# nianticlabs/map-free-reloc

Measured on AMD Instinct MI355X. Metric: image-pairs/sec @ 540x720 (SuperPoint+SuperGlue + PnP w/ depth), higher is better.
Workload: dtype f32 in / f32 accumulate; matrix products of the 3x3 convolutions, attention, the transformer's linear layers and SuperPoint's 1x1 descriptor head on the f16 matrix cores with every fp32 operand carried as TWO f16 terms (xh = rne_f16(x), xl = rne_f16((x - xh) 2^11); weights pre-scaled per output feat

## Files before the change

include/mfr_hip.h:

```cpp
#ifndef MFR_HIP_H
#define MFR_HIP_H
#include <stddef.h>
#include <stdint.h>

#ifdef __cplusplus
extern "C" {
#endif

#define MFR_ABI_VERSION 6

#define MFR_K_F32 0
#define MFR_K_F64 1

#define MFR_E_ARG      (-1)
#define MFR_E_LAUNCH   (-2)
#define MFR_E_WORKSPACE (-3)

#define MFR_ST_OK          0
#define MFR_ST_TOO_FEW     1
#define MFR_ST_BAD_DEPTH   2
#define MFR_ST_NO_MODEL    3
#define MFR_ST_DEGENERATE  4

int mfr_abi_version(void);

int mfr_f16x2_guard_bind(int *device_flag);
#define MFR_ST_RANGE 7
const char *mfr_target_arch(void);

int mfr_test_f64_ops(const double *a, const double *b, const double *c, int n, double *out3, void *stream);
int mfr_test_sample(uint64_t seed, const int64_t *pair_ids, int B, int iters, int n, int k, int32_t *out, void *stream);

size_t mfr_pnp_workspace_bytes(int B, int maxN, int max_iters);
int mfr_pnp_solve_batch(const float *pts0, const float *pts1, const int32_t *n_corr, int B, int maxN,
                        const float *depth0, int H, int W,
                        const void *K0, const void *K1, int k_dtype,
                        int max_iters, double reproj_thr, double confidence,
                        uint64_t seed, const int64_t *pair_ids,
                        void *workspace, size_t workspace_bytes,
                        double *R, double *t, int32_t *n_inliers, int32_t *status, uint8_t *inlier_mask,
                        void *stream);

int mfr_depth_min(const float *depth, int B, int H, int W, float *partial_min , void *stream);
int mfr_pnp_lift(const float *pts0, const float *pts1, const int32_t *n_corr, int B, int maxN,
                 const float *depth0, const float *partial_min, int H, int W, const void *K0, int k_dtype,
                 double *xyz, double *obs, int32_t *src_idx, int32_t *n_valid, void *stream);
int mfr_pnp_ransac(const double *xyz, const double *obs, const int32_t *n_valid, int B, int maxN,
                   const void *K1, int k_dtype, int max_iters, double reproj_thr, double confidence,
                   uint64_t seed, const int64_t *pair_ids,
                   int32_t *counts , int32_t *inl_idx ,
                   double *R, double *t, int32_t *n_inliers, int32_t *status,
                   uint8_t *mask_valid ,
                   int32_t *best_iter , int32_t *iters_run ,
                   void *stream);

size_t mfr_rig_pnp_workspace_bytes(int B, int T, int maxN, int max_iters);
int mfr_rig_pnp_ransac(const double *xyz, const double *obs, const int32_t *n_valid, int B, int T, int maxN,
                       const void *K1, int k_dtype, const double *rig, int max_iters, double reproj_thr, double confidence,
                       uint64_t seed, const int64_t *pair_ids,
                       int32_t *counts , int32_t *inl_idx ,
                       double *R, double *t, int32_t *n_inliers, int32_t *status,
                       uint8_t *mask_valid ,
                       int32_t *best_iter , int32_t *iters_run ,
                       void *stream);
int mfr_rig_pnp_solve_batch(const float *pts0, const float *pts1, const int32_t *n_corr, int B, int T, int maxN,
                            const float *depth0, int H, int W,
                            const void *K0, const void *K1, int k_dtype, const double *rig,
                            int max_iters, double reproj_thr, double confidence,
                            uint64_t seed, const int64_t *pair_ids,
                            void *workspace, size_t workspace_bytes,
                            double *R, double *t, int32_t *n_inliers, int32_t *status, uint8_t *inlier_mask ,
                            void *stream);

size_t mfr_scale_workspace_bytes(int B, int maxN);
int mfr_scale_from_depth_batch(const float *pts0, const float *pts1, const uint8_t *emat_mask,
                               const int32_t *n_corr, int B, int maxN,
                               const float *depth0, const float *depth1, int H, int W,
                               const void *K0, const void *K1, int k_dtype,
                               const double *R, const double *t,
                               const int32_t *in_status ,
                               double scale_thr,
                               void *workspace, size_t workspace_bytes,
                               double *t_metric, double *best_scale, int32_t *n_inliers, int32_t *status,
                               void *stream);

#define MFR_AP_OK            0
#define MFR_AP_APPROXIMATED  1
#define MFR_AP_NO_PAIRS      2
#define MFR_AP_TOO_MANY      3
#define MFR_AP_BAD_OFFSETS   4
#define MFR_AP_ITER_CAP      16
#define MFR_AP_MAX_PAIRS     64
#define MFR_AP_MAX_LO_ITERS  62
#define MFR_AP_WEISZFELD_CAP 256
size_t mfr_abs_pose_workspace_bytes(int P);
int mfr_abs_pose_fuse(const double *train_q, const double *train_c, const double *pred_R, const double *pred_t, int P,
                      const int32_t *offsets, int Q, int mode, double thr_deg, double thr_mult, int lo_iters, uint64_t seed,
                      void *workspace, size_t workspace_bytes,
                      double *abs_q, double *abs_c, int32_t *inlier_mask, int32_t *status, void *stream);
int mfr_test_abs_pose_subset(uint64_t seed, const uint64_t *base, int n, int calls, int iters, int nsub, uint64_t *out, void *stream);

#define MFR_EMAT_SCORE_MAGSAC 0
#define MFR_EMAT_SCORE_COUNT  1
#define MFR_MAGSAC_LUT_M 2048
int mfr_magsac_lut(double *lut_host , int M);
size_t mfr_emat_workspace_bytes(int B, int maxN, int max_iters);
int mfr_emat_solve_batch(const float *pts0, const float *pts1, const int32_t *n_corr, int B, int maxN,
                         const void *K0, const void *K1, int k_dtype, double pix_thr, double confidence, int max_iters,
                         uint64_t seed, const int64_t *pair_ids, int score_method, const double *magsac_lut, int lut_m,
                         double max_thr_ratio, void *workspace, size_t workspace_bytes,
                         double *R, double *t, int32_t *n_inliers, int32_t *status, uint8_t *inlier_mask,
                         int32_t *best_iter, int32_t *iters_run, int32_t *counts_out, double *losses_out, int32_t *lo_runs,
                         void *stream);

size_t mfr_procrustes_workspace_bytes(int B, int maxN, int max_iters);
int mfr_procrustes_solve_batch(const float *pts0, const float *pts1, const int32_t *n_corr, int B, int maxN,
                               const float *depth0, const float *depth1, int H, int W, const void *K0, const void *K1, int k_dtype,
                               double max_corr_dist, double confidence, int max_iters, uint64_t seed, const int64_t *pair_ids,
                               void *workspace, size_t workspace_bytes, double *R, double *t, int32_t *n_inliers,
                               int32_t *status, int32_t *best_iter, int32_t *iters_run, int32_t *counts_out, void *stream);

int mfr_sp_scoremap(const float *logits, int B, int Hc, int Wc, float *scores, void *stream);
int mfr_sp_nms_candidates(const float *scores, int B, int H, int W, int nms_radius, float threshold, int border,
                          float *nms_out, uint64_t *cand, int cand_cap, int32_t *cand_count, void *stream);
int mfr_sp_select_topk(const uint64_t *cand, int cand_cap, const int32_t *cand_count, int B, int W, int K,
                       float *kpts, float *kscores, int32_t *n_kpts, void *stream);
int mfr_sp_sample_descriptors(const float *dense_nhwc, int B, int Hc, int Wc, const float *kpts,
                              const int32_t *n_kpts, int K, float *desc, void *stream);

size_t mfr_gemm_f16x2_pack_bytes(int N, int K);
int mfr_gemm_f16x2_pack(const float *w, int N, int K, void *packed, void *stream);
int mfr_gemm_f16x2(const float *x, int ldx, const void *packed_w, const float *bias, float *y, int ldy, int M, int N, int K, int flags, void *stream);
int mfr_gemm_f16x2_pack_batched(const float *w, int ldw, int nbatch, long long w_batch_stride, int N, int K, float out_mul, void *packed, void *stream);
int mfr_gemm_f16x2_batched(const float *x, int ldx, long long x_batch_stride, const void *packed_w, const float *bias, float *y, int ldy, long long y_batch_stride,
                           int nbatch, int M, int N, int K, int flags, void *stream);
int mfr_conv_igemm_k(int Cin, int KH, int KW);
int mfr_conv_igemm_f16x2(const float *x, const void *packed_w, const float *bias, float *y, int B, int Cin, int H, int W, int Cout, int KH, int KW,
                         int stride, int pad, int relu, void *stream);
int mfr_conv_igemm_f16x2_pad(const float *x, const void *packed_w, const float *bias, float *y, int B, int Cin, int H, int W, int Cout, int KH, int KW,
                             int stride, int pad_lo, int pad_hi, int relu, void *stream);
int mfr_conv_igemm_f16x2_upadd(const float *x, const void *packed_w, const float *bias, const float *lo, int Hl, int Wl, float *y, int B, int Cin, int H, int W,
                               int Cout, int KH, int KW, int stride, int pad, void *stream);
int mfr_gemm_f16x2_ln(const float *x, int ldx, const void *packed_w, const float *bias, const float *gamma, const float *beta, float eps, float *y, int ldy,
                      int M, int N, int K, int accumulate, void *stream);
int mfr_gemm_bf16x3_ln(const float *x, int ldx, const void *packed_w, const float *bias, const float *gamma, const float *beta, float eps, float *y, int ldy,
                       int M, int N, int K, int accumulate, void *stream);
int mfr_gemm_f16x2_windows(const float *feat, int Bimg, int Hf, int Wf, int C, const int32_t *img_ids, const int32_t *cell_ids, int nwin, int wc, int stride, int win,
                           const float *zero_row, const void *packed_w, const float *bias, const float *window_bias, float *y, int ldy, int N, void *stream);
int mfr_gemm_bf16x3_windows(const float *feat, int Bimg, int Hf, int Wf, int C, const int32_t *img_ids, const int32_t *cell_ids, int nwin, int wc, int stride, int win,
                            const float *zero_row, const void *packed_w, const float *bias, const float *window_bias, float *y, int ldy, int N, void *stream);
int mfr_mlp_ln_f16x2(const float *x, int ldx, int K1, const void *packed_w1, const float *b1, const void *packed_w2, const float *b2, const float *gamma, const float *beta,
                     float eps, float *y, int ldy, int M, int accumulate, void *stream);
int mfr_mlp_ln_bf16x3(const float *x, int ldx, int K1, const void *packed_w1, const float *b1, const void *packed_w2, const float *b2, const float *gamma, const float *beta,
                      float eps, float *y, int ldy, int M, int accumulate, void *stream);
size_t mfr_gemm_bf16x3_pack_bytes(int N, int K);
int mfr_gemm_bf16x3_pack(const float *w, int N, int K, void *packed, void *stream);
int mfr_gemm_bf16x3(const float *x, int ldx, const void *packed_w, const float *bias, float *y, int ldy, int M, int N, int K, int flags, void *stream);
int mfr_sg_attention(const float *q, const float *k, const float *v, int ld, int B2, int N, int heads,
                     const int32_t *n_tok, int cross, float *out, int ldo, void *stream);
int mfr_sg_attention_variant(const float *q, const float *k, const float *v, int ld, int B2, int N, int heads,
                             const int32_t *n_tok, int cross, float *out, int ldo, int variant, void *stream);
size_t mfr_sg_match_workspace_bytes(int B, int ldS);
int mfr_sg_sinkhorn_match(const float *S, int B, int ldS, const int32_t *n0, const int32_t *n1,
                          float bin_score, int iters, float match_thr,
                          const float *kpts0, const float *kpts1, int K,
                          void *workspace, size_t workspace_bytes,
                          int32_t *matches0, float *mscores0, float *pts0, float *pts1, int maxN, int32_t *n_corr,
                          void *stream);
int mfr_sg_sinkhorn_match_variant(const float *S, int B, int ldS, const int32_t *n0, const int32_t *n1,
                                  float bin_score, int iters, float match_thr,
                                  const float *kpts0, const float *kpts1, int K,
                                  void *workspace, size_t workspace_bytes,
                                  int32_t *matches0, float *mscores0, float *pts0, float *pts1, int maxN, int32_t *n_corr,
                                  int variant, void *stream);

int mfr_gemm_f16x2_ln_gelu(const float *x, int ldx, const void *packed_w, const float *bias, const float *gamma, const float *beta, float eps, float *y, int ldy,
                           int M, int N, int K, void *stream);
int mfr_gemm_bf16x3_ln_gelu(const float *x, int ldx, const void *packed_w, const float *bias, const float *gamma, const float *beta, float eps, float *y, int ldy,
                            int M, int N, int K, void *stream);
int mfr_lg_rotary_table(const float *kpts_norm, const float *wr, int M, float *cs, void *stream);
int mfr_lg_rotary_apply(float *q, float *k, int ld, int M, const float *cs, void *stream);
int mfr_lg_ln_gelu(float *x, int ld, int M, const float *gamma, const float *beta, float eps, void *stream);
size_t mfr_lg_assign_workspace_bytes(int B, int N0, int N1);
int mfr_lg_assign(const float *S, int B, int N0, int N1, int ldS, const float *z0, const float *z1, const int32_t *n0, const int32_t *n1,
                  float threshold, const float *kpts0, const float *kpts1, int K, void *workspace, size_t workspace_bytes,
                  int32_t *matches0, int32_t *matches1, float *mscores0, float *mscores1, float *pts0, float *pts1, int maxN, int32_t *n_corr,
                  void *stream);

size_t mfr_loftr_linear_attention_workspace_bytes(int B, int L, int heads);
int mfr_loftr_linear_attention(const float *q, int ldq, const float *k, const float *v, int ld, int B, int L, int heads,
                               void *workspace, size_t workspace_bytes, float *out, int ldo, void *stream);
int mfr_loftr_fine_attention(const float *q, int ldq, const float *k, const float *v, int ld, int Bw, int L, int D, int heads,
                             float *out, int ldo, void *stream);
size_t mfr_loftr_coarse_match_workspace_bytes(int B, int L0, int L1);
int mfr_loftr_coarse_match(const float *S, int B, int h0, int w0, int h1, int w1, float temperature, float thr, int border,
                           void *workspace, size_t workspace_bytes, int32_t *i_ids, int32_t *j_ids, float *mconf,
                           int32_t *n_match, void *stream);
int mfr_loftr_coarse_match_variant(const float *S, int B, int h0, int w0, int h1, int w1, float temperature, float thr, int border,
                                   void *workspace, size_t workspace_bytes, int32_t *i_ids, int32_t *j_ids, float *mconf,
                                   int32_t *n_match, int variant, void *stream);
size_t mfr_loftr_ot_match_workspace_bytes(int B, int L0, int L1);
int mfr_loftr_ot_match(const float *S, int B, int h0, int w0, int h1, int w1, float bin_score, int iters, float thr, int border,
                       void *workspace, size_t workspace_bytes, int32_t *i_ids, int32_t *j_ids, float *mconf, int32_t *n_match,
                       float *u_out, float *v_out, int variant, void *stream);
int mfr_loftr_gather_windows(const float *feat, int Bimg, int Hf, int Wf, int C, const int32_t *img_ids,
                             const int32_t *cell_ids, int M, int wc, int stride, int win, float *out, void *stream);
int mfr_loftr_fine_match(const float *g0, const float *g1, int ld, int C, int M, int W, float out_scale, const int32_t *lin_idx,
                         const float *k1, float *pts1, float *expec, void *stream);

int mfr_conv3x3_c1_relu(const float *x, const float *w, const float *bias, int B, int H, int W, int out_channels,
                        float *y, void *stream);
int mfr_bias_relu_nchw(float *x, const float *bias, int B, int C, int HW, void *stream);
int mfr_conv1x1_nchw(const float *x, const float *w, const float *bias, int B, int Cin, int Cout, int HW, float *y, void *stream);
int mfr_nchw_to_rows(const float *x, const float *add, int B, int C, int HW, int deinterleave, float *out, long long out_img_stride, int ldo, void *stream);
int mfr_nchw_to_rows_gather(const float *x, const float *add, int n_src, int C, int HW, const int32_t *idx, int n_out, float *out, long long out_img_stride,
                            int ldo, void *stream);
int mfr_bias_pool2_relu_nchw(const float *x, const float *bias, int B, int C, int H, int W, float *y, void *stream);

size_t mfr_procrustes_icp_workspace_bytes(int B, int H, int W);
int mfr_procrustes_icp_refine(const float *depth0, const float *depth1, int B, int H, int W, const void *K0, const void *K1, int k_dtype,
                              double max_corr_dist, double rel_fitness, double rel_rmse, int max_iter, const int32_t *status,
                              void *workspace, size_t workspace_bytes, double *R, double *t, int32_t *n_inliers, double *fitness,
                              double *rmse, int32_t *iters, void *stream);

int mfr_layernorm(const float *x, int ldx, const float *gamma, const float *beta, const float *residual, int ldr, long long rows, int C,
                  float eps, float *out, int ldo, void *stream);
int mfr_upsample2x_add(const float *lo, float *y, int planes, int H, int W, void *stream);
int mfr_upsample_bilinear(const void *in, void *out, int planes, int H, int W, int Ho, int Wo, int dtype, void *stream);
int mfr_conv_gemm_bf16(const void *A, long long sA, const long long *segA, const void *B, long long sB, const long long *segB,
                       int Lk, int nkc_total, int nkc_z, const float *bias, void *C, long long ldc, int out_dtype,
                       int M, int N, int nz, const long long *zA, const long long *zB, const long long *zC, const int *zk, void *stream);
int mfr_conv_pack_nhwc_halo(const void *x, int x_dtype, int B, int C, int H, int W, int Wp, void *out, int guard_rows, void *stream);
int mfr_conv_pack_cm_halo(const void *x, int x_dtype, long long BC, int H, int W, int Wq, long long L, int ncopies, int first_shift, long long slack,
                          void *out, void *stream);
int mfr_conv_unpack_nchw(const void *haloed, int B, int N, int H, int W, int Wp, void *y, void *stream);

int mfr_kabsch_fwd(const float *H, int B, float *R, void *stream);
int mfr_kabsch_bwd(const float *H, const float *gR, int B, float *gH, void *stream);

int mfr_rootsift(const float *desc, int n_rows, float *out, float *norm2, void *stream);
int mfr_desc_ratio_match(const float *des0, const float *des1, const float *norm0, const float *norm1,
                         const float *kp0, const float *kp1, int B, int N0, int N1,
                         const int32_t *n0, const int32_t *n1, double ratio,
                         int32_t *nn_idx, float *nn_d2, float *pts0, float *pts1, int maxN, int32_t *n_corr,
                         void *stream);

#define MFR_SIFT_ST_CAND_OVERFLOW 1
#define MFR_SIFT_ST_KPT_OVERFLOW  2
#define MFR_SIFT_ST_OUT_OVERFLOW  4
size_t mfr_sift_workspace_bytes(int B, int H, int W, int cand_cap);
long long mfr_sift_level_offset(int B, int H, int W, int octave, int level, int *Ho_host, int *Wo_host);
int mfr_sift_blur_taps(int level, float *taps_host, int *radius_host);
int mfr_sift_detect(const uint8_t *gray, int B, int H, int W, int nfeatures, int Nmax, int cand_cap, void *workspace,
                    size_t workspace_bytes, float *kpts, float *desc, float *size, float *angle, float *response,
                    int32_t *octave, int32_t *n, int32_t *status, void *stream);

size_t mfr_jpeg_workspace_bytes(int n, int H, int W, long long max_record_bytes, int subseq_bits);
int mfr_jpeg_decode(const void *headers, const uint8_t *records, const long long *offsets, int n, int H, int W,
                    long long max_record_bytes, float *gray, uint8_t *rgb, int32_t *status, int32_t *rounds, void *workspace,
                    size_t workspace_bytes, int subseq_bits, void *stream);

size_t mfr_png_depth_workspace_bytes(int n, int H, int W);
int mfr_png_depth_decode(const void *headers, const uint8_t *records, const long long *offsets, int n, int H, int W,
                         long long max_record_bytes, void *scratch, size_t scratch_bytes, float *out, int32_t *status, void *stream);

int mfr_resize_gray_bilinear(const uint8_t *rgb, int n, int H, int W, const int32_t *status,
                             const int32_t *y0, const int32_t *y1, const float *fy,
                             const int32_t *x0, const int32_t *x1, const float *fx,
                             int h, int w, float *out, void *stream);

size_t mfr_wino_f16x2_filter_bytes(int Cin, int Cout);
int mfr_wino_f16x2_filter_transform(const float *w, int Cin, int Cout, void *upk, void *stream);
int mfr_conv3x3_wino_f16x2(const float *x, const void *upk, const float *bias, const float *residual, int B, int Cin, int Cout,
                           int H, int W, int act, int pool, float *y, void *stream);
size_t mfr_conv3x3_direct_f16x2_filter_bytes(int Cin, int Cout);
int mfr_conv3x3_direct_f16x2_filter_pack(const float *w, int Cin, int Cout, void *packed, void *stream);
int mfr_conv3x3_direct_f16x2(const float *x, const void *packed, const float *bias, const float *residual, int B, int Cin, int Cout,
                             int H, int W, int act, int pool, float *y, void *stream);
int mfr_conv3x3_direct_f16x2_rows(const float *x, const void *packed, const float *bias, int B, int Cin, int Cout, int H, int W, int act, float *yrows, int ldy, void *stream);
int mfr_conv3x3_direct_f16x2_tiled(const float *x, const void *packed, const float *bias, const float *residual, int B, int Cin, int Cout, int H, int W,
                                   int act, int pool, float *y, int ldrows, int tile_mode, int pitch, void *stream);
int mfr_conv3x3s2_direct_f16x2(const float *x, const void *packed, const float *bias, int B, int Cin, int Cout, int H, int W, int act, float *y, void *stream);
int mfr_sp_conv1ab_f16x2(const float *gray, const float *w1a, const float *b1a, const void *upk1b, const float *bias1b, int B, int H, int W, float *y, void *stream);
size_t mfr_wino_bf16x3_filter_bytes(int Cin, int Cout);
int mfr_wino_bf16x3_filter_transform(const float *w, int Cin, int Cout, void *upk, void *stream);
int mfr_conv3x3_wino_bf16x3(const float *x, const void *upk, const float *bias, const float *residual, int B, int Cin, int Cout,
                            int H, int W, int act, int pool, float *y, void *stream);
size_t mfr_wino_filter_bytes(int Cin, int Cout);
int mfr_wino_filter_transform(const float *w, int Cin, int Cout, float *upk, void *stream);
int mfr_conv3x3_wino(const float *x, const float *upk, const float *bias, const float *residual, int B, int Cin, int Cout,
                     int H, int W, int act, int pool, float *y, void *stream);
int mfr_conv3x3_wino_variant(const float *x, const float *upk, const float *bias, const float *residual, int B, int Cin, int Cout,
                             int H, int W, int act, int pool, int variant, float *y, void *stream);

int mfr_corr_warp_fwd(const float *q, const float *k, const float *v, const float *grid, int B, int Dq, int N,
                      float *warped, float *pos, float *max_score, float *row_max, float *row_sum, void *stream);
int mfr_corr_warp_bwd(const float *q, const float *k, const float *v, const float *grid, int B, int Dq, int N,
                      const float *d_warped, const float *d_pos, const float *d_max, const float *delta,
                      const float *row_max, const float *row_sum, float *dq, float *dk, float *dv, void *stream);

int mfr_dpt_prep(const void *img, int dtype, int B, int H, int W, float *out, int Hn, int Wn, void *stream);
int mfr_dpt_groupnorm(const float *x, const float *gamma, const float *beta, const float *residual, int B, int C, int HW, int G, float eps, int relu,
                      float *y, void *stream);
int mfr_dpt_maxpool3s2(const float *x, int planes, int H, int W, int pad_top, int pad_bottom, int pad_left, int pad_right, float *y, void *stream);
int mfr_dpt_layernorm(const float *x, int ldx, const float *gamma, const float *beta, const float *residual, int ldr, long long rows, int C, float eps,
                      float *out, int ldo, void *stream);
int mfr_dpt_bias_gelu(float *x, int ld, long long rows, int N, const float *bias, void *stream);
int mfr_dpt_add_relu(const float *a, const float *b, long long n, float *sum, float *relu_out, void *stream);
int mfr_dpt_tokens(const float *x, const float *cls, const float *pos, int B, int C, int HW, float *out, int ldo, void *stream);
int mfr_dpt_tokens_inverse(const float *rows, int ld, long long img_stride, int skip, const float *bias_img, int gelu, int B, int C, int HW, float *out,
                           void *stream);
int mfr_dpt_shuffle(const float *g, int ld, const float *bias, int B, int C, int H, int W, int s, float *out, void *stream);
int mfr_dpt_head_tail(const float *f, const float *w, float bias, int B, int C, int Hh, int Wh, int invert, float scale, float shift, int Ho, int Wo,
                      float *metres, uint16_t *mm, void *stream);
int mfr_dpt_prep_rows(const uint8_t *img, int N, const int *rows, int m, int H, int W, float *out, int Hn, int Wn, int *status, void *stream);
int mfr_dpt_head_tail_rows(const float *f, const float *w, float bias, int B, int C, int Hh, int Wh, int invert, float scale, float shift, int Ho, int Wo,
                           const int *src, const int *dst, int d, float *metres, uint16_t *mm, int D, int quantize, int *status, void *stream);

int mfr_eloftr_stem_s2(const float *x, const float *w, const float *bias, int B, int H, int W, int out_channels, float *y, void *stream);
int mfr_eloftr_aggregate(const float *x, int ldx, long long img_stride, int nimg, int hc, int wc, const float *wq, const float *gamma, const float *beta, float eps,
                         float *q_out, float *kv_out, void *stream);
int mfr_eloftr_rotary(float *q, float *k, int ld, const float *cos_sin, long long rows, int La, void *stream);
int mfr_eloftr_attention(const float *q, int ldq, const float *k, const float *v, int ldkv, int nb, int Lq, int Lk, int heads, float *out, int ldo, void *stream);
int mfr_eloftr_upsample4_rows(const float *msg, int ldm, int nimg, int ha, int wa, float *dst, int ldx, long long img_stride, void *stream);
int mfr_eloftr_upsample2x(const float *in, const float *add, float *out, int planes, int H, int W, void *stream);
int mfr_eloftr_leaky_relu(float *x, int ld, long long rows, int N, float slope, void *stream);
int mfr_eloftr_rows_to_nchw(const float *x, int ldx, long long img_stride, int nimg, int C, int HW, float scale, float *out, void *stream);
int mfr_eloftr_gather_windows(const float *feat_half, int nimg, int Hh, int Wh, int C, const int32_t *img_ids, const int32_t *cell_ids, long long ld_cells,
                              const int32_t *n, int B, int maxN, int wc, int cell_px, int win, int pad, float *out, void *stream);
int mfr_eloftr_fine_match(const float *win0, const float *win1, const int32_t *cell_i, const int32_t *cell_j, long long ld_cells, const int32_t *n, int B, int maxN,
                          int wc, int cell_px, float *pts0, float *pts1, int32_t *stage1_arg, void *stream);
int mfr_eloftr_compact(const float *pts0, const float *pts1, const float *conf, long long ld_conf, const int32_t *n, int B, int maxN, int W, int H, float *out0,
                       float *out1, float *out_conf, int32_t *n_out, void *stream);

#ifdef __cplusplus
}
#endif
#endif
```

map-free-reloc_amd/_lib.py:

```python
import ctypes as C
import os

_HERE = os.path.dirname(os.path.abspath(__file__))
SO_PATH = os.path.join(_HERE, "csrc", "libmfr_hip.so")

_lib = None

_vp, _i, _d, _u64, _sz = C.c_void_p, C.c_int, C.c_double, C.c_uint64, C.c_size_t

SIGNATURES = {
    "mfr_abi_version": (_i, []),
    "mfr_target_arch": (C.c_char_p, []),
    "mfr_f16x2_guard_bind": (_i, [_vp]),
    "mfr_test_f64_ops": (_i, [_vp, _vp, _vp, _i, _vp, _vp]),
    "mfr_test_sample": (_i, [_u64, _vp, _i, _i, _i, _i, _vp, _vp]),
    "mfr_pnp_workspace_bytes": (_sz, [_i, _i, _i]),
    "mfr_pnp_solve_batch": (_i, [_vp, _vp, _vp, _i, _i, _vp, _i, _i, _vp, _vp, _i, _i, _d, _d, _u64, _vp,
                                 _vp, _sz, _vp, _vp, _vp, _vp, _vp, _vp]),
    "mfr_depth_min": (_i, [_vp, _i, _i, _i, _vp, _vp]),
    "mfr_pnp_lift": (_i, [_vp, _vp, _vp, _i, _i, _vp, _vp, _i, _i, _vp, _i, _vp, _vp, _vp, _vp, _vp]),
    "mfr_pnp_ransac": (_i, [_vp, _vp, _vp, _i, _i, _vp, _i, _i, _d, _d, _u64, _vp, _vp, _vp, _vp, _vp, _vp, _vp,
                            _vp, _vp, _vp, _vp]),
    "mfr_rig_pnp_workspace_bytes": (_sz, [_i, _i, _i, _i]),
    "mfr_rig_pnp_ransac": (_i, [_vp, _vp, _vp, _i, _i, _i, _vp, _i, _vp, _i, _d, _d, _u64, _vp, _vp, _vp, _vp, _vp, _vp, _vp,
                                _vp, _vp, _vp, _vp]),
    "mfr_rig_pnp_solve_batch": (_i, [_vp, _vp, _vp, _i, _i, _i, _vp, _i, _i, _vp, _vp, _i, _vp, _i, _d, _d, _u64, _vp,
                                     _vp, _sz, _vp, _vp, _vp, _vp, _vp, _vp]),
    "mfr_emat_workspace_bytes": (_sz, [_i, _i, _i]),
    "mfr_magsac_lut": (_i, [_vp, _i]),
    "mfr_emat_solve_batch": (_i, [_vp, _vp, _vp, _i, _i, _vp, _vp, _i, _d, _d, _i, _u64, _vp, _i, _vp, _i, _d, _vp, _sz,
                                  _vp, _vp, _vp, _vp, _vp, _vp, _vp, _vp, _vp, _vp, _vp]),
    "mfr_procrustes_workspace_bytes": (_sz, [_i, _i, _i]),
    "mfr_procrustes_solve_batch": (_i, [_vp, _vp, _vp, _i, _i, _vp, _vp, _i, _i, _vp, _vp, _i, _d, _d, _i, _u64, _vp, _vp, _sz,
                                        _vp, _vp, _vp, _vp, _vp, _vp, _vp, _vp]),
    "mfr_procrustes_icp_workspace_bytes": (_sz, [_i, _i, _i]),
    "mfr_procrustes_icp_refine": (_i, [_vp, _vp, _i, _i, _i, _vp, _vp, _i, _d, _d, _d, _i, _vp, _vp, _sz, _vp, _vp, _vp, _vp, _vp, _vp, _vp]),
    "mfr_sp_scoremap": (_i, [_vp, _i, _i, _i, _vp, _vp]),
    "mfr_sp_nms_candidates": (_i, [_vp, _i, _i, _i, _i, C.c_float, _i, _vp, _vp, _i, _vp, _vp]),
    "mfr_sp_select_topk": (_i, [_vp, _i, _vp, _i, _i, _i, _vp, _vp, _vp, _vp]),
    "mfr_sp_sample_descriptors": (_i, [_vp, _i, _i, _i, _vp, _vp, _i, _vp, _vp]),
    "mfr_gemm_f16x2_pack_bytes": (_sz, [_i, _i]),
    "mfr_gemm_f16x2_pack": (_i, [_vp, _i, _i, _vp, _vp]),
    "mfr_gemm_f16x2": (_i, [_vp, _i, _vp, _vp, _vp, _i, _i, _i, _i, _i, _vp]),
    "mfr_gemm_f16x2_pack_batched": (_i, [_vp, _i, _i, C.c_longlong, _i, _i, C.c_float, _vp, _vp]),
    "mfr_gemm_f16x2_batched": (_i, [_vp, _i, C.c_longlong, _vp, _vp, _vp, _i, C.c_longlong, _i, _i, _i, _i, _i, _vp]),
    "mfr_conv_igemm_k": (_i, [_i, _i, _i]),
    "mfr_conv_igemm_f16x2": (_i, [_vp, _vp, _vp, _vp, _i, _i, _i, _i, _i, _i, _i, _i, _i, _i, _vp]),
    "mfr_conv_igemm_f16x2_pad": (_i, [_vp, _vp, _vp, _vp, _i, _i, _i, _i, _i, _i, _i, _i, _i, _i, _i, _vp]),
    "mfr_conv_igemm_f16x2_upadd": (_i, [_vp, _vp, _vp, _vp, _i, _i, _vp, _i, _i, _i, _i, _i, _i, _i, _i, _i, _vp]),
    "mfr_gemm_f16x2_windows": (_i, [_vp, _i, _i, _i, _i, _vp, _vp, _i, _i, _i, _i, _vp, _vp, _vp, _vp, _vp, _i, _i, _vp]),
    "mfr_gemm_bf16x3_windows": (_i, [_vp, _i, _i, _i, _i, _vp, _vp, _i, _i, _i, _i, _vp, _vp, _vp, _vp, _vp, _i, _i, _vp]),
    "mfr_mlp_ln_f16x2": (_i, [_vp, _i, _i, _vp, _vp, _vp, _vp, _vp, _vp, C.c_float, _vp, _i, _i, _i, _vp]),
    "mfr_mlp_ln_bf16x3": (_i, [_vp, _i, _i, _vp, _vp, _vp, _vp, _vp, _vp, C.c_float, _vp, _i, _i, _i, _vp]),
    "mfr_gemm_f16x2_ln": (_i, [_vp, _i, _vp, _vp, _vp, _vp, C.c_float, _vp, _i, _i, _i, _i, _i, _vp]),
    "mfr_gemm_bf16x3_ln": (_i, [_vp, _i, _vp, _vp, _vp, _vp, C.c_float, _vp, _i, _i, _i, _i, _i, _vp]),
    "mfr_gemm_bf16x3_pack_bytes": (_sz, [_i, _i]),
    "mfr_gemm_bf16x3_pack": (_i, [_vp, _i, _i, _vp, _vp]),
    "mfr_gemm_bf16x3": (_i, [_vp, _i, _vp, _vp, _vp, _i, _i, _i, _i, _i, _vp]),
    "mfr_sg_attention": (_i, [_vp, _vp, _vp, _i, _i, _i, _i, _vp, _i, _vp, _i, _vp]),
    "mfr_sg_attention_variant": (_i, [_vp, _vp, _vp, _i, _i, _i, _i, _vp, _i, _vp, _i, _i, _vp]),
    "mfr_sg_match_workspace_bytes": (_sz, [_i, _i]),
    "mfr_sg_sinkhorn_match": (_i, [_vp, _i, _i, _vp, _vp, C.c_float, _i, C.c_float, _vp, _vp, _i, _vp, _sz,
                                   _vp, _vp, _vp, _vp, _i, _vp, _vp]),
    "mfr_sg_sinkhorn_match_variant": (_i, [_vp, _i, _i, _vp, _vp, C.c_float, _i, C.c_float, _vp, _vp, _i, _vp, _sz,
                                           _vp, _vp, _vp, _vp, _i, _vp, _i, _vp]),
    "mfr_gemm_f16x2_ln_gelu": (_i, [_vp, _i, _vp, _vp, _vp, _vp, C.c_float, _vp, _i, _i, _i, _i, _vp]),
    "mfr_gemm_bf16x3_ln_gelu": (_i, [_vp, _i, _vp, _vp, _vp, _vp, C.c_float, _vp, _i, _i, _i, _i, _vp]),
    "mfr_lg_rotary_table": (_i, [_vp, _vp, _i, _vp, _vp]),
    "mfr_lg_rotary_apply": (_i, [_vp, _vp, _i, _i, _vp, _vp]),
    "mfr_lg_ln_gelu": (_i, [_vp, _i, _i, _vp, _vp, C.c_float, _vp]),
    "mfr_lg_assign_workspace_bytes": (_sz, [_i, _i, _i]),
    "mfr_lg_assign": (_i, [_vp, _i, _i, _i, _i, _vp, _vp, _vp, _vp, C.c_float, _vp, _vp, _i, _vp, _sz,
                           _vp, _vp, _vp, _vp, _vp, _vp, _i, _vp, _vp]),
    "mfr_loftr_linear_attention_workspace_bytes": (_sz, [_i, _i, _i]),
    "mfr_loftr_linear_attention": (_i, [_vp, _i, _vp, _vp, _i, _i, _i, _i, _vp, _sz, _vp, _i, _vp]),
    "mfr_loftr_coarse_match_workspace_bytes": (_sz, [_i, _i, _i]),
    "mfr_loftr_coarse_match": (_i, [_vp, _i, _i, _i, _i, _i, C.c_float, C.c_float, _i, _vp, _sz, _vp, _vp, _vp, _vp, _vp]),
    "mfr_loftr_ot_match_workspace_bytes": (_sz, [_i, _i, _i]),
    "mfr_loftr_ot_match": (_i, [_vp, _i, _i, _i, _i, _i, C.c_float, _i, C.c_float, _i, _vp, _sz, _vp, _vp, _vp, _vp, _vp, _vp, _i, _vp]),
    "mfr_loftr_coarse_match_variant": (_i, [_vp, _i, _i, _i, _i, _i, C.c_float, C.c_float, _i, _vp, _sz, _vp, _vp, _vp, _vp, _i, _vp]),
    "mfr_loftr_fine_attention": (_i, [_vp, _i, _vp, _vp, _i, _i, _i, _i, _i, _vp, _i, _vp]),
    "mfr_loftr_gather_windows": (_i, [_vp, _i, _i, _i, _i, _vp, _vp, _i, _i, _i, _i, _vp, _vp]),
    "mfr_loftr_fine_match": (_i, [_vp, _vp, _i, _i, _i, _i, C.c_float, _vp, _vp, _vp, _vp, _vp]),
    "mfr_conv3x3_c1_relu": (_i, [_vp, _vp, _vp, _i, _i, _i, _i, _vp, _vp]),
    "mfr_bias_relu_nchw": (_i, [_vp, _vp, _i, _i, _i, _vp]),
    "mfr_conv1x1_nchw": (_i, [_vp, _vp, _vp, _i, _i, _i, _i, _vp, _vp]),
    "mfr_nchw_to_rows": (_i, [_vp, _vp, _i, _i, _i, _i, _vp, C.c_longlong, _i, _vp]),
    "mfr_nchw_to_rows_gather": (_i, [_vp, _vp, _i, _i, _i, _vp, _i, _vp, C.c_longlong, _i, _vp]),
    "mfr_bias_pool2_relu_nchw": (_i, [_vp, _vp, _i, _i, _i, _i, _vp, _vp]),
    "mfr_wino_bf16x3_filter_bytes": (_sz, [_i, _i]),
    "mfr_wino_bf16x3_filter_transform": (_i, [_vp, _i, _i, _vp, _vp]),
    "mfr_conv3x3_wino_bf16x3": (_i, [_vp, _vp, _vp, _vp, _i, _i, _i, _i, _i, _i, _i, _vp, _vp]),
    "mfr_sp_conv1ab_f16x2": (_i, [_vp, _vp, _vp, _vp, _vp, _i, _i, _i, _vp, _vp]),
    "mfr_wino_f16x2_filter_bytes": (_sz, [_i, _i]),
    "mfr_wino_f16x2_filter_transform": (_i, [_vp, _i, _i, _vp, _vp]),
    "mfr_conv3x3_wino_f16x2": (_i, [_vp, _vp, _vp, _vp, _i, _i, _i, _i, _i, _i, _i, _vp, _vp]),
    "mfr_conv3x3_direct_f16x2_filter_bytes": (_sz, [_i, _i]),
    "mfr_conv3x3_direct_f16x2_filter_pack": (_i, [_vp, _i, _i, _vp, _vp]),
    "mfr_conv3x3_direct_f16x2": (_i, [_vp, _vp, _vp, _vp, _i, _i, _i, _i, _i, _i, _i, _vp, _vp]),
    "mfr_conv3x3s2_direct_f16x2": (_i, [_vp, _vp, _vp, _i, _i, _i, _i, _i, _i, _vp, _vp]),
    "mfr_conv3x3_direct_f16x2_rows": (_i, [_vp, _vp, _vp, _i, _i, _i, _i, _i, _i, _vp, _i, _vp]),
    "mfr_conv3x3_direct_f16x2_tiled": (_i, [_vp, _vp, _vp, _vp, _i, _i, _i, _i, _i, _i, _i, _vp, _i, _i, _i, _vp]),
    "mfr_wino_filter_bytes": (_sz, [_i, _i]),
    "mfr_wino_filter_transform": (_i, [_vp, _i, _i, _vp, _vp]),
    "mfr_conv3x3_wino": (_i, [_vp, _vp, _vp, _vp, _i, _i, _i, _i, _i, _i, _i, _vp, _vp]),
    "mfr_conv3x3_wino_variant": (_i, [_vp, _vp, _vp, _vp, _i, _i, _i, _i, _i, _i, _i, _i, _vp, _vp]),
    "mfr_layernorm": (_i, [_vp, _i, _vp, _vp, _vp, _i, C.c_longlong, _i, C.c_float, _vp, _i, _vp]),
    "mfr_conv_gemm_bf16": (_i, [_vp, C.c_longlong, _vp, _vp, C.c_longlong, _vp, _i, _i, _i, _vp, _vp, C.c_longlong, _i,
                                _i, _i, _i, _vp, _vp, _vp, _vp, _vp]),
    "mfr_conv_pack_nhwc_halo": (_i, [_vp, _i, _i, _i, _i, _i, _i, _vp, _i, _vp]),
    "mfr_conv_unpack_nchw": (_i, [_vp, _i, _i, _i, _i, _i, _vp, _vp]),
    "mfr_conv_pack_cm_halo": (_i, [_vp, _i, C.c_longlong, _i, _i, _i, C.c_longlong, _i, _i, C.c_longlong, _vp, _vp]),
    "mfr_upsample2x_add": (_i, [_vp, _vp, _i, _i, _i, _vp]),
    "mfr_upsample_bilinear": (_i, [_vp, _vp, _i, _i, _i, _i, _i, _i, _vp]),
    "mfr_corr_warp_fwd": (_i, [_vp, _vp, _vp, _vp, _i, _i, _i, _vp, _vp, _vp, _vp, _vp, _vp]),
    "mfr_corr_warp_bwd": (_i, [_vp, _vp, _vp, _vp, _i, _i, _i, _vp, _vp, _vp, _vp, _vp, _vp, _vp, _vp, _vp, _vp]),
    "mfr_kabsch_fwd": (_i, [_vp, _i, _vp, _vp]),
    "mfr_kabsch_bwd": (_i, [_vp, _vp, _i, _vp, _vp]),
    "mfr_rootsift": (_i, [_vp, _i, _vp, _vp, _vp]),
    "mfr_desc_ratio_match": (_i, [_vp, _vp, _vp, _vp, _vp, _vp, _i, _i, _i, _vp, _vp, _d, _vp, _vp, _vp, _vp, _i, _vp, _vp]),
    "mfr_sift_workspace_bytes": (_sz, [_i, _i, _i, _i]),
    "mfr_sift_level_offset": (C.c_longlong, [_i, _i, _i, _i, _i, _vp, _vp]),
    "mfr_sift_blur_taps": (_i, [_i, _vp, _vp]),
    "mfr_sift_detect": (_i, [_vp, _i, _i, _i, _i, _i, _i, _vp, _sz, _vp, _vp, _vp, _vp, _vp, _vp, _vp, _vp, _vp]),
    "mfr_jpeg_workspace_bytes": (_sz, [_i, _i, _i, C.c_longlong, _i]),
    "mfr_jpeg_decode": (_i, [_vp, _vp, _vp, _i, _i, _i, C.c_longlong, _vp, _vp, _vp, _vp, _vp, _sz, _i, _vp]),
    "mfr_png_depth_workspace_bytes": (_sz, [_i, _i, _i]),
    "mfr_png_depth_decode": (_i, [_vp, _vp, _vp, _i, _i, _i, C.c_longlong, _vp, _sz, _vp, _vp, _vp]),
    "mfr_resize_gray_bilinear": (_i, [_vp, _i, _i, _i, _vp, _vp, _vp, _vp, _vp, _vp, _vp, _i, _i, _vp, _vp]),
    "mfr_scale_workspace_bytes": (_sz, [_i, _i]),
    "mfr_scale_from_depth_batch": (_i, [_vp, _vp, _vp, _vp, _i, _i, _vp, _vp, _i, _i, _vp, _vp, _i, _vp, _vp, _vp,
                                        _d, _vp, _sz, _vp, _vp, _vp, _vp, _vp]),
    "mfr_abs_pose_workspace_bytes": (_sz, [_i]),
    "mfr_test_abs_pose_subset": (_i, [_u64, _vp, _i, _i, _i, _i, _vp, _vp]),
    "mfr_abs_pose_fuse": (_i, [_vp, _vp, _vp, _vp, _i, _vp, _i, _i, _d, _d, _i, _u64, _vp, _sz, _vp, _vp, _vp, _vp, _vp]),
    "mfr_dpt_prep": (_i, [_vp, _i, _i, _i, _i, _vp, _i, _i, _vp]),
    "mfr_dpt_groupnorm": (_i, [_vp, _vp, _vp, _vp, _i, _i, _i, _i, C.c_float, _i, _vp, _vp]),
    "mfr_dpt_maxpool3s2": (_i, [_vp, _i, _i, _i, _i, _i, _i, _i, _vp, _vp]),
    "mfr_dpt_layernorm": (_i, [_vp, _i, _vp, _vp, _vp, _i, C.c_longlong, _i, C.c_float, _vp, _i, _vp]),
    "mfr_dpt_bias_gelu": (_i, [_vp, _i, C.c_longlong, _i, _vp, _vp]),
    "mfr_dpt_add_relu": (_i, [_vp, _vp, C.c_longlong, _vp, _vp, _vp]),
    "mfr_dpt_tokens": (_i, [_vp, _vp, _vp, _i, _i, _i, _vp, _i, _vp]),
    "mfr_dpt_tokens_inverse": (_i, [_vp, _i, C.c_longlong, _i, _vp, _i, _i, _i, _i, _vp, _vp]),
    "mfr_dpt_shuffle": (_i, [_vp, _i, _vp, _i, _i, _i, _i, _i, _vp, _vp]),
    "mfr_dpt_head_tail": (_i, [_vp, _vp, C.c_float, _i, _i, _i, _i, _i, C.c_float, C.c_float, _i, _i, _vp, _vp, _vp]),
    "mfr_dpt_prep_rows": (_i, [_vp, _i, _vp, _i, _i, _i, _vp, _i, _i, _vp, _vp]),
    "mfr_dpt_head_tail_rows": (_i, [_vp, _vp, C.c_float, _i, _i, _i, _i, _i, C.c_float, C.c_float, _i, _i, _vp, _vp, _i, _vp, _vp, _i, _i, _vp, _vp]),
    "mfr_eloftr_stem_s2": (_i, [_vp, _vp, _vp, _i, _i, _i, _i, _vp, _vp]),
    "mfr_eloftr_aggregate": (_i, [_vp, _i, C.c_longlong, _i, _i, _i, _vp, _vp, _vp, C.c_float, _vp, _vp, _vp]),
    "mfr_eloftr_rotary": (_i, [_vp, _vp, _i, _vp, C.c_longlong, _i, _vp]),
    "mfr_eloftr_attention": (_i, [_vp, _i, _vp, _vp, _i, _i, _i, _i, _i, _vp, _i, _vp]),
    "mfr_eloftr_upsample4_rows": (_i, [_vp, _i, _i, _i, _i, _vp, _i, C.c_longlong, _vp]),
    "mfr_eloftr_upsample2x": (_i, [_vp, _vp, _vp, _i, _i, _i, _vp]),
    "mfr_eloftr_leaky_relu": (_i, [_vp, _i, C.c_longlong, _i, C.c_float, _vp]),
    "mfr_eloftr_rows_to_nchw": (_i, [_vp, _i, C.c_longlong, _i, _i, _i, C.c_float, _vp, _vp]),
    "mfr_eloftr_gather_windows": (_i, [_vp, _i, _i, _i, _i, _vp, _vp, C.c_longlong, _vp, _i, _i, _i, _i, _i, _i, _vp, _vp]),
    "mfr_eloftr_fine_match": (_i, [_vp, _vp, _vp, _vp, C.c_longlong, _vp, _i, _i, _i, _i, _vp, _vp, _vp, _vp]),
    "mfr_eloftr_compact": (_i, [_vp, _vp, _vp, C.c_longlong, _vp, _i, _i, _i, _i, _vp, _vp, _vp, _vp, _vp]),
}


class MfrLibraryError(RuntimeError):
    pass


def load(require_gpu=False):
    global _lib
    if _lib is None:
        import torch
        if not os.path.exists(SO_PATH):
            raise MfrLibraryError(
                f"{SO_PATH} not found: build it with `python -c 'import __graft_entry__ as g; g.build()'` "
                f"(hipcc --offload-arch=gfx950).  There is no CPU fallback.")
        lib = C.CDLL(SO_PATH)
        for name, (res, args) in SIGNATURES.items():
            try:
                fn = getattr(lib, name)
            except AttributeError as e:
                raise MfrLibraryError(f"libmfr_hip.so does not export {name}") from e
            fn.restype = res
            fn.argtypes = args
        _lib = lib
    if require_gpu:
        import torch
        if not torch.cuda.is_available():
            raise MfrLibraryError("no HIP device visible: the HIP path cannot run (there is no CPU fallback)")
    return _lib


def check(rc, what):
    if rc != 0:
        raise MfrLibraryError(f"{what} failed with code {rc} (see include/mfr_hip.h MFR_E_*)")


def ptr(t):
    if t is None:
        return None
    assert t.is_contiguous(), "C-ABI needs contiguous buffers"
    return t.data_ptr()


def stream_ptr():
    import torch
    return torch.cuda.current_stream().cuda_stream
```

map-free-reloc_amd/csrc/attention.hip:

```cpp
#include <hip/hip_runtime.h>
#include <math.h>
#include <stdint.h>

#include "../../include/mfr_hip.h"
#include "wave_dev.h"
#include "split_f16.h"
#include "guard.h"

typedef float f32x16 __attribute__((ext_vector_type(16)));

#define AT_D 64
#define AT_KT 32
#define AT_KS 68
#define AT_QW 32
#define AT_WAVES 4

__device__ __forceinline__ void at_store_zero_row(float *row)
{
#pragma unroll
    for (int g = 0; g < 8; ++g) ((float4 *)row)[g] = make_float4(0.f, 0.f, 0.f, 0.f);
}
__device__ __forceinline__ void at_store_normalised(float *op, f32x16 o0, f32x16 o1, float inv)
{
#pragma unroll
    for (int g = 0; g < 4; ++g) {
        *(float4 *)(op + 8 * g) = make_float4(o0[4 * g] * inv, o0[4 * g + 1] * inv, o0[4 * g + 2] * inv, o0[4 * g + 3] * inv);
        *(float4 *)(op + 32 + 8 * g) = make_float4(o1[4 * g] * inv, o1[4 * g + 1] * inv, o1[4 * g + 2] * inv, o1[4 * g + 3] * inv);
    }
}

__global__ void __launch_bounds__(256, 2) sg_attention_kernel(
    const float *__restrict__ Q, const float *__restrict__ Kp, const float *__restrict__ Vp, int ld,
    int N, int heads, int B2, const int *__restrict__ n_tok, int cross, float scale_log2e, float *__restrict__ O, int ldo)
{
    __shared__ __attribute__((aligned(16))) float Ks[2][AT_KT][AT_KS];
    __shared__ __attribute__((aligned(16))) float Vs[2][AT_KT][AT_D];
    const int nbh = heads * B2;
    const int bh = blockIdx.x % nbh, qb = blockIdx.x / nbh;
    const int b = bh / heads, h = bh - b * heads;
    const int bk = cross ? (b ^ 1) : b;
    const int tid = threadIdx.x, lane = tid & 63, wid = tid >> 6;
    const int ql = lane & 31, half = lane >> 5;
    const int nq = n_tok[b], nk = n_tok[bk];
    const int q0 = qb * (AT_QW * AT_WAVES);
    const int q = q0 + wid * AT_QW + ql;
    if (q0 >= nq) {
        if (q < N) at_store_zero_row(O + ((size_t)b * N + q) * ldo + h * AT_D + 32 * half);
        return;
    }

    float qreg[32];
    {
        const bool ok = q < N;
        const float4 *qp = (const float4 *)(Q + ((size_t)b * N + (ok ? q : 0)) * ld + h * AT_D + half * 32);
#pragma unroll
        for (int g = 0; g < 8; ++g) {
            float4 t = ok ? qp[g] : make_float4(0.f, 0.f, 0.f, 0.f);
            qreg[4 * g] = t.x * scale_log2e; qreg[4 * g + 1] = t.y * scale_log2e;
            qreg[4 * g + 2] = t.z * scale_log2e; qreg[4 * g + 3] = t.w * scale_log2e;
        }
    }
    f32x16 o0, o1;
#pragma unroll
    for (int r = 0; r < 16; ++r) { o0[r] = 0.f; o1[r] = 0.f; }
    float m_run = -INFINITY, l_run = 0.f;

    const int sr = tid >> 4, sc = (tid & 15) * 4;
    const float *kbase = Kp + (size_t)bk * N * ld + h * AT_D + sc;
    const float *vbase = Vp + (size_t)bk * N * ld + h * AT_D + sc;
    const int ntiles = (nk + AT_KT - 1) / AT_KT;
    float4 kr0, kr1, vr0, vr1;
    auto gload = [&](int t) {
        const int k0 = t * AT_KT + sr, k1 = k0 + 16;
        const float4 z = make_float4(0.f, 0.f, 0.f, 0.f);
        kr0 = (k0 < nk) ? *(const float4 *)(kbase + (size_t)k0 * ld) : z;
        kr1 = (k1 < nk) ? *(const float4 *)(kbase + (size_t)k1 * ld) : z;
        vr0 = (k0 < nk) ? *(const float4 *)(vbase + (size_t)k0 * ld) : z;
        vr1 = (k1 < nk) ? *(const float4 *)(vbase + (size_t)k1 * ld) : z;
    };
    auto lstore = [&](int buf) {
        *(float4 *)&Ks[buf][sr][sc] = kr0; *(float4 *)&Ks[buf][sr + 16][sc] = kr1;
        *(float4 *)&Vs[buf][sr][sc] = vr0; *(float4 *)&Vs[buf][sr + 16][sc] = vr1;
    };
    if (ntiles > 0) { gload(0); lstore(0); }
    __syncthreads();

    for (int t = 0; t < ntiles; ++t) {
        const int buf = t & 1;
        if (t + 1 < ntiles) gload(t + 1);

        f32x16 s;
#pragma unroll
        for (int r = 0; r < 16; ++r) s[r] = 0.f;
        const float *krow = &Ks[buf][ql][half * 32];
#pragma unroll
        for (int g = 0; g < 8; ++g) {
            const float4 a = *(const float4 *)(krow + 4 * g);
            s = __builtin_amdgcn_mfma_f32_32x32x2f32(a.x, qreg[4 * g], s, 0, 0, 0);
            s = __builtin_amdgcn_mfma_f32_32x32x2f32(a.y, qreg[4 * g + 1], s, 0, 0, 0);
            s = __builtin_amdgcn_mfma_f32_32x32x2f32(a.z, qreg[4 * g + 2], s, 0, 0, 0);
            s = __builtin_amdgcn_mfma_f32_32x32x2f32(a.w, qreg[4 * g + 3], s, 0, 0, 0);
        }
        const int kb = t * AT_KT + 4 * half;
        float mx = -INFINITY;
#pragma unroll
        for (int r = 0; r < 16; ++r) {
            const int key = kb + (r & 3) + 8 * (r >> 2);
            if (key >= nk) s[r] = -INFINITY;
            mx = fmaxf(mx, s[r]);
        }
        mx = fmaxf(mx, __shfl_xor(mx, 32, 64));
        const float m_new = fmaxf(m_run, mx);
        const float alpha = __builtin_amdgcn_exp2f(m_run - m_new);
        float rs = 0.f;
#pragma unroll
        for (int r = 0; r < 16; ++r) { s[r] = __builtin_amdgcn_exp2f(s[r] - m_new); rs += s[r]; }
        rs += __shfl_xor(rs, 32, 64);
        l_run = l_run * alpha + rs;
        m_run = m_new;
#pragma unroll
        for (int r = 0; r < 16; ++r) { o0[r] *= alpha; o1[r] *= alpha; }
#pragma unroll
        for (int r = 0; r < 16; ++r) {
            const int key = 4 * half + (r & 3) + 8 * (r >> 2);
            const float a0 = Vs[buf][key][ql], a1 = Vs[buf][key][32 + ql];
            o0 = __builtin_amdgcn_mfma_f32_32x32x2f32(a0, s[r], o0, 0, 0, 0);
            o1 = __builtin_amdgcn_mfma_f32_32x32x2f32(a1, s[r], o1, 0, 0, 0);
        }
        if (t + 1 < ntiles) lstore(buf ^ 1);
        __syncthreads();
    }

    if (q < N) {
        const float inv = (l_run > 0.f && q < nq) ? 1.f / l_run : 0.f;
        at_store_normalised(O + ((size_t)b * N + q) * ldo + h * AT_D + 4 * half, o0, o1, inv);
    }
}


typedef short bf16x8 __attribute__((ext_vector_type(8)));

#define AB_KS 72
#define AB_VS 40
#define AB_WAVES 8

typedef float at_f2 __attribute__((ext_vector_type(2)));
union Frag8 { bf16x8 v; unsigned u[4]; uint4 q; };

#define MFMA_BF16(a, b, c) __builtin_amdgcn_mfma_f32_32x32x16_bf16((a).v, (b).v, (c), 0, 0, 0)
#define AT_BF16X3_QK(kf, qf, s, s2) do { \
        s2 = MFMA_BF16(kf[1], qf[1], s2); s = MFMA_BF16(kf[0], qf[2], s); s2 = MFMA_BF16(kf[2], qf[0], s2); \
        s = MFMA_BF16(kf[0], qf[1], s); s2 = MFMA_BF16(kf[1], qf[0], s2); s = MFMA_BF16(kf[0], qf[0], s); } while (0)
#define AT_BF16X3_PV(vf, pf, o0, o1) do { \
        o0 = MFMA_BF16(vf[2], pf[1], o0); o1 = MFMA_BF16(vf[3], pf[1], o1); o0 = MFMA_BF16(vf[0], pf[2], o0); o1 = MFMA_BF16(vf[1], pf[2], o1); \
        o0 = MFMA_BF16(vf[4], pf[0], o0); o1 = MFMA_BF16(vf[5], pf[0], o1); o0 = MFMA_BF16(vf[0], pf[1], o0); o1 = MFMA_BF16(vf[1], pf[1], o1); \
        o0 = MFMA_BF16(vf[2], pf[0], o0); o1 = MFMA_BF16(vf[3], pf[0], o1); o0 = MFMA_BF16(vf[0], pf[0], o0); o1 = MFMA_BF16(vf[1], pf[0], o1); } while (0)
struct AtBf16x3 {
    static constexpr int NT = 3, NO = 1;
    static constexpr bool WEAVE = true, GUARD = false, P_COPY = true;
    template <class W> static __device__ __forceinline__ void split2(float x0f, float x1f, W &&word)
    {
        at_f2 x; x.x = x0f; x.y = x1f;
        const unsigned x0 = __float_as_uint(x.x), x1 = __float_as_uint(x.y);
        at_f2 h; h.x = __uint_as_float(x0 & 0xffff0000u); h.y = __uint_as_float(x1 & 0xffff0000u);
        const at_f2 r = x - h;
        const unsigned r0 = __float_as_uint(r.x), r1 = __float_as_uint(r.y);
        at_f2 m; m.x = __uint_as_float(r0 & 0xffff0000u); m.y = __uint_as_float(r1 & 0xffff0000u);
        const at_f2 l = r - m;
        word(0) = bf_pack_hi16(x0, x1); word(1) = bf_pack_hi16(r0, r1); word(2) = bf_pack_hi16(__float_as_uint(l.x), __float_as_uint(l.y));
    }
    static __device__ __forceinline__ float fold(float main, float second) { return main + second; }
};

#define MFMA_F16(a, b, c) SF_MFMA((a).q, (b).q, (c))
#define AT_F16X2_QK(kf, qf, s, s2) do { s2 = MFMA_F16(kf[0], qf[1], s2); s = MFMA_F16(kf[0], qf[0], s); s2 = MFMA_F16(kf[1], qf[0], s2); } while (0)
#define AT_F16X2_PV(vf, pf, o0, o1, c0, c1) do { \
        c0 = MFMA_F16(vf[0], pf[1], c0); c1 = MFMA_F16(vf[1], pf[1], c1); o0 = MFMA_F16(vf[0], pf[0], o0); o1 = MFMA_F16(vf[1], pf[0], o1); \
        c0 = MFMA_F16(vf[2], pf[0], c0); c1 = MFMA_F16(vf[3], pf[0], c1); } while (0)
struct AtF16x2 {
    static constexpr int NT = 2, NO = 2;
    static constexpr bool WEAVE = false, GUARD = true, P_COPY = false;
    template <class W> static __device__ __forceinline__ void split2(float x0, float x1, W &&word) { sf_split2(x0, x1, SF_LOW_SCALE, word(0), word(1)); }
    static __device__ __forceinline__ float fold(float main, float second) { return __builtin_fmaf(second, 1.0f / SF_LOW_SCALE, main); }
};

template <class AR>
__device__ __forceinline__ void sg_attention_split_p(
    const float *Q, const float *Kp, const float *Vp, int ld, int N, int heads, int B2, const int *n_tok, int cross, float scale_log2e, float *O, int ldo, int *guard)
{
    constexpr int NT = AR::NT, NO = AR::NO;
    __shared__ __attribute__((aligned(16))) unsigned short Ks[2][NT][AT_KT][AB_KS];
    __shared__ __attribute__((aligned(16))) unsigned short Vt[2][NT][AT_D][AB_VS];
    const int nbh = heads * B2;
    const int bh = blockIdx.x % nbh, qb = blockIdx.x / nbh;
    const int b = bh / heads, h = bh - b * heads;
    const int bk = cross ? (b ^ 1) : b;
    const int tid = threadIdx.x, lane = tid & 63, wid = __builtin_amdgcn_readfirstlane(tid >> 6);
    const int ql = lane & 31, half = lane >> 5;
    const int nq = n_tok[b], nk = n_tok[bk];
    const int q0 = qb * (AT_QW * AB_WAVES);
    const int q = q0 + wid * AT_QW + ql;
    if (q0 >= nq) {
        if (q < N) at_store_zero_row(O + ((size_t)b * N + q) * ldo + h * AT_D + 32 * half);
        return;
    }

    Frag8 qf[4][NT];
    {
        const bool ok = q < N;
        const float *qp = Q + ((size_t)b * N + (ok ? q : 0)) * ld + h * AT_D + half * 8;
#pragma unroll
        for (int s = 0; s < 4; ++s) {
            float4 t0 = *(const float4 *)(qp + 16 * s), t1 = *(const float4 *)(qp + 16 * s + 4);
            if (!ok) { t0 = make_float4(0.f, 0.f, 0.f, 0.f); t1 = t0; }
            AR::split2(t0.x * scale_log2e, t0.y * scale_log2e, [&](int k) -> unsigned & { return qf[s][k].u[0]; });
            AR::split2(t0.z * scale_log2e, t0.w * scale_log2e, [&](int k) -> unsigned & { return qf[s][k].u[1]; });
            AR::split2(t1.x * scale_log2e, t1.y * scale_log2e, [&](int k) -> unsigned & { return qf[s][k].u[2]; });
            AR::split2(t1.z * scale_log2e, t1.w * scale_log2e, [&](int k) -> unsigned & { return qf[s][k].u[3]; });
        }
    }
    f32x16 o0, o1, c0, c1;
#pragma unroll
    for (int r = 0; r < 16; ++r) { o0[r] = 0.f; o1[r] = 0.f; c0[r] = 0.f; c1[r] = 0.f; }
    float m_run = -INFINITY, l_run = 0.f;

    const int sr = tid >> 4, sc4 = (tid & 15) * 4;
    const unsigned rowb = (unsigned)ld * 4u;
    const unsigned span = nk > 0 ? (unsigned)(nk - 1) * rowb + AT_D * 4u : 0u;
    const __amdgpu_buffer_rsrc_t rk = __builtin_amdgcn_make_buffer_rsrc((void *)(Kp + (size_t)bk * N * ld + h * AT_D), 0, (int)span, MFR_RSRC_FLAGS);
    const __amdgpu_buffer_rsrc_t rv = __builtin_amdgcn_make_buffer_rsrc((void *)(Vp + (size_t)bk * N * ld + h * AT_D), 0, (int)span, MFR_RSRC_FLAGS);
    const unsigned koff = (unsigned)sr * rowb + 4u * (unsigned)sc4, voff = 4u * (unsigned)lane;
    const int ntiles = (nk + AT_KT - 1) / AT_KT;
    float4 kr;
    float v0, v1, v2, v3;
    auto gload_k = [&](int t) { kr = __builtin_bit_cast(float4, __builtin_amdgcn_raw_buffer_load_b128(rk, koff, (unsigned)(t * AT_KT) * rowb, 0)); };
    auto gload_v = [&](int t) {
        const unsigned sv = (unsigned)(t * AT_KT + 4 * wid) * rowb;
        v0 = __builtin_bit_cast(float, __builtin_amdgcn_raw_buffer_load_b32(rv, voff, sv, 0));
        v1 = __builtin_bit_cast(float, __builtin_amdgcn_raw_buffer_load_b32(rv, voff, sv + rowb, 0));
        v2 = __builtin_bit_cast(float, __builtin_amdgcn_raw_buffer_load_b32(rv, voff, sv + 2u * rowb, 0));
        v3 = __builtin_bit_cast(float, __builtin_amdgcn_raw_buffer_load_b32(rv, voff, sv + 3u * rowb, 0));
    };
    auto lstore_k = [&](int buf) {
        unsigned w[NT][2];
        AR::split2(kr.x, kr.y, [&](int k) -> unsigned & { return w[k][0]; }); AR::split2(kr.z, kr.w, [&](int k) -> unsigned & { return w[k][1]; });
        *(uint2 *)&Ks[buf][0][sr][sc4] = make_uint2(w[0][0], w[0][1]); *(uint2 *)&Ks[buf][1][sr][sc4] = make_uint2(w[1][0], w[1][1]);
        if constexpr (NT == 3) *(uint2 *)&Ks[buf][2][sr][sc4] = make_uint2(w[2][0], w[2][1]);
    };
    auto lstore_v = [&](int buf) {
        unsigned w[NT][2];
        AR::split2(v0, v1, [&](int k) -> unsigned & { return w[k][0]; }); AR::split2(v2, v3, [&](int k) -> unsigned & { return w[k][1]; });
        const int p0 = 16 * (wid >> 2) + 8 * (wid & 1) + 4 * ((wid >> 1) & 1);
        *(uint2 *)&Vt[buf][0][lane][p0] = make_uint2(w[0][0], w[0][1]); *(uint2 *)&Vt[buf][1][lane][p0] = make_uint2(w[1][0], w[1][1]);
        if constexpr (NT == 3) *(uint2 *)&Vt[buf][2][lane][p0] = make_uint2(w[2][0], w[2][1]);
    };
    const unsigned short *kq0 = &Ks[0][0][ql][8 * half], *vq0 = &Vt[0][0][ql][8 * half];
#define AT_KLOAD(f, kq, st) do { f[0].q = *(const uint4 *)((kq) + 16 * (st)); f[1].q = *(const uint4 *)((kq) + AT_KT * AB_KS + 16 * (st)); \
        if constexpr (NT == 3) f[2].q = *(const uint4 *)((kq) + 2 * AT_KT * AB_KS + 16 * (st)); } while (0)
#define AT_VLOAD(f, vq, st) do { \
        f[0].q = *(const uint4 *)((vq) + 16 * (st)); f[1].q = *(const uint4 *)((vq) + 32 * AB_VS + 16 * (st)); \
        f[2].q = *(const uint4 *)((vq) + AT_D * AB_VS + 16 * (st)); f[3].q = *(const uint4 *)((vq) + AT_D * AB_VS + 32 * AB_VS + 16 * (st)); \
        if constexpr (NT == 3) { f[4].q = *(const uint4 *)((vq) + 2 * AT_D * AB_VS + 16 * (st)); f[5].q = *(const uint4 *)((vq) + 2 * AT_D * AB_VS + 32 * AB_VS + 16 * (st)); } } while (0)
#define AT_WEAVE(nm, nv) do { if constexpr (AR::WEAVE) { _Pragma("unroll") for (int w_ = 0; w_ < (nm); ++w_) { \
        __builtin_amdgcn_sched_group_barrier(0x8, 1, 0); __builtin_amdgcn_sched_group_barrier(0x2, (nv), 0); } } } while (0)
#define AT_QK(kf, qf, s, s2) do { if constexpr (NT == 3) AT_BF16X3_QK(kf, qf, s, s2); else AT_F16X2_QK(kf, qf, s, s2); } while (0)
#define AT_PV(vf, pf) do { if constexpr (NT == 3) AT_BF16X3_PV(vf, pf, o0, o1); else AT_F16X2_PV(vf, pf, o0, o1, c0, c1); } while (0)
#define AT_SPLIT_P(pf, o) do { if constexpr (AR::P_COPY) { \
            float pp_[8]; \
            _Pragma("unroll") for (int j_ = 0; j_ < 8; ++j_) pp_[j_] = p[(o) + j_]; \
            _Pragma("unroll") for (int j_ = 0; j_ < 4; ++j_) AR::split2(pp_[2 * j_], pp_[2 * j_ + 1], [&](int k) -> unsigned & { return pf[k].u[j_]; }); \
        } else { \
            _Pragma("unroll") for (int j_ = 0; j_ < 4; ++j_) AR::split2(p[(o) + 2 * j_], p[(o) + 2 * j_ + 1], [&](int k) -> unsigned & { return pf[k].u[j_]; }); \
        } } while (0)
#define AT_FOLD_SCORES(sc, s, s2) do { _Pragma("unroll") for (int r_ = 0; r_ < 16; ++r_) sc[r_] = AR::fold(s[r_], s2[r_]); } while (0)

    f32x16 sc;
    gload_k(0); gload_v(0); lstore_k(0); lstore_v(0);
    gload_k(1); lstore_k(1);
    gload_k(2); gload_v(1);
    __syncthreads();
    {
        f32x16 s, s2;
#pragma unroll
        for (int r = 0; r < 16; ++r) { s[r] = 0.f; s2[r] = 0.f; }
        if (ntiles > 0) {
#pragma unroll
            for (int st = 0; st < 4; ++st) { Frag8 kf[NT]; AT_KLOAD(kf, kq0, st); AT_QK(kf, qf[st], s, s2); }
        }
        AT_FOLD_SCORES(sc, s, s2);
    }
    __syncthreads();

    for (int t = 0; t < ntiles; ++t) {
        const int buf = t & 1;
        const unsigned short *kq = kq0 + (buf ^ 1) * (NT * AT_KT * AB_KS);
        const unsigned short *vq = vq0 + buf * (NT * AT_D * AB_VS);
        f32x16 s, s2;
#pragma unroll
        for (int r = 0; r < 16; ++r) { s[r] = 0.f; s2[r] = 0.f; }
        Frag8 ka[NT], kb2[NT];
        AT_KLOAD(ka, kq, 0);
        AT_KLOAD(kb2, kq, 1);
        const int kb = t * AT_KT + 4 * half;
        if ((t + 1) * AT_KT > nk) {
#pragma unroll
            for (int r = 0; r < 16; ++r)
                if (kb + (r & 3) + 8 * (r >> 2) >= nk) sc[r] = -INFINITY;
        }
        AT_QK(ka, qf[0], s, s2);
        AT_KLOAD(ka, kq, 2);
        float mx = sc[0];
#pragma unroll
        for (int r = 1; r < 15; r += 2) mx = fmaxf(fmaxf(mx, sc[r]), sc[r + 1]);
        mx = fmaxf(mx, sc[15]);
        mx = fmaxf(mx, __shfl_xor(mx, 32, 64));
        const float m_new = fmaxf(m_run, mx);
        AT_WEAVE(6, 2);
        __builtin_amdgcn_sched_barrier(0);
        AT_QK(kb2, qf[1], s, s2);
        AT_KLOAD(kb2, kq, 3);
        float p[16];
        at_f2 rs2; rs2.x = 0.f; rs2.y = 0.f;
        at_f2 mm; mm.x = m_new; mm.y = m_new;
#pragma unroll
        for (int r = 0; r < 8; r += 2) {
            at_f2 d; d.x = sc[r]; d.y = sc[r + 1];
            d = d - mm;
            at_f2 e; e.x = __builtin_amdgcn_exp2f(d.x); e.y = __builtin_amdgcn_exp2f(d.y);
            rs2 += e;
            p[r] = e.x; p[r + 1] = e.y;
        }
        AT_WEAVE(6, 3);
        __builtin_amdgcn_sched_barrier(0);
        AT_QK(ka, qf[2], s, s2);
#pragma unroll
        for (int r = 8; r < 16; r += 2) {
            at_f2 d; d.x = sc[r]; d.y = sc[r + 1];
            d = d - mm;
            at_f2 e; e.x = __builtin_amdgcn_exp2f(d.x); e.y = __builtin_amdgcn_exp2f(d.y);
            rs2 += e;
            p[r] = e.x; p[r + 1] = e.y;
        }
        float rs = rs2.x + rs2.y;
        rs += __shfl_xor(rs, 32, 64);
        AT_WEAVE(6, 3);
        __builtin_amdgcn_sched_barrier(0);
        if (__ballot(m_new != m_run) != 0ull) {
            const float alpha = __builtin_amdgcn_exp2f(m_run - m_new);
            l_run *= alpha;
#pragma unroll
            for (int r = 0; r < 16; ++r) { o0[r] *= alpha; o1[r] *= alpha; c0[r] *= alpha; c1[r] *= alpha; }
        }
        l_run += rs;
        m_run = m_new;
        AT_QK(kb2, qf[3], s, s2);
        Frag8 va[2 * NT];
        AT_VLOAD(va, vq, 0);
        Frag8 pf0[NT];
        AT_SPLIT_P(pf0, 0);
        lstore_k(buf); lstore_v(buf ^ 1);
        gload_k(t + 3); gload_v(t + 2);
        AT_WEAVE(6, 14);
        __builtin_amdgcn_sched_barrier(0);
        AT_PV(va, pf0);
        Frag8 vb[2 * NT];
        AT_VLOAD(vb, vq, 1);
        Frag8 pf1[NT];
        AT_SPLIT_P(pf1, 8);
        AT_WEAVE(12, 4);
        __builtin_amdgcn_sched_barrier(0);
        AT_PV(vb, pf1);
        AT_FOLD_SCORES(sc, s, s2);
        __syncthreads();
    }
#undef AT_FOLD_SCORES
#undef AT_SPLIT_P
#undef AT_PV
#undef AT_QK
#undef AT_WEAVE
#undef AT_VLOAD
#undef AT_KLOAD

    if (q < N) {
        const float inv = (l_run > 0.f && q < nq) ? 1.f / l_run : 0.f;
        float *op = O + ((size_t)b * N + q) * ldo + h * AT_D + 4 * half;
        if constexpr (AR::GUARD) {
            if (guard) {
                float chk = 0.f;
#pragma unroll
                for (int r = 0; r < 16; ++r) { MFR_GUARD_ACC(chk, o0[r]); MFR_GUARD_ACC(chk, c0[r]); MFR_GUARD_ACC(chk, o1[r]); MFR_GUARD_ACC(chk, c1[r]); }
                MFR_GUARD_ACC(chk, l_run);
                if (chk != chk) atomicOr(guard, 1);
            }
        }
        if constexpr (NO == 2) {
#pragma unroll
            for (int r = 0; r < 16; ++r) { o0[r] = AR::fold(o0[r], c0[r]); o1[r] = AR::fold(o1[r], c1[r]); }
        }
        at_store_normalised(op, o0, o1, inv);
    }
}

__global__ void __launch_bounds__(512, 1) sg_attention_bf16x3_p_kernel(
    const float *__restrict__ Q, const float *__restrict__ Kp, const float *__restrict__ Vp, int ld,
    int N, int heads, int B2, const int *__restrict__ n_tok, int cross, float scale_log2e, float *__restrict__ O, int ldo)
{
    sg_attention_split_p<AtBf16x3>(Q, Kp, Vp, ld, N, heads, B2, n_tok, cross, scale_log2e, O, ldo, nullptr);
}

__global__ void __launch_bounds__(512, 1) sg_attention_f16x2_p_kernel(
    const float *__restrict__ Q, const float *__restrict__ Kp, const float *__restrict__ Vp, int ld,
    int N, int heads, int B2, const int *__restrict__ n_tok, int cross, float scale_log2e, float *__restrict__ O, int ldo, int *guard)
{
    sg_attention_split_p<AtF16x2>(Q, Kp, Vp, ld, N, heads, B2, n_tok, cross, scale_log2e, O, ldo, guard);
}

extern "C" {

int mfr_sg_attention_variant(const float *q, const float *k, const float *v, int ld, int B2, int N, int heads,
                             const int32_t *n_tok, int cross, float *out, int ldo, int variant, void *stream)
{
    if (!q || !k || !v || !n_tok || !out || B2 <= 0 || N <= 0 || heads <= 0 || (ld & 3) || (ldo & 3)) return MFR_E_ARG;
    if (cross && (B2 & 1)) return MFR_E_ARG;
    if (variant < 0 || variant > 2) return MFR_E_ARG;
    if (variant != 1 && (size_t)N * ld * 4 >= 0x7fffffffull) variant = 1;
    const float scale_log2e = 1.4426950408889634f / 8.0f;
    if (variant != 1) {
        const int nqb = (N + AT_QW * AB_WAVES - 1) / (AT_QW * AB_WAVES);
        if (variant == 0)
            hipLaunchKernelGGL(sg_attention_f16x2_p_kernel, dim3(nqb * heads * B2), dim3(512), 0, (hipStream_t)stream, q, k, v, ld, N, heads, B2, n_tok, cross,
                               scale_log2e, out, ldo, mfr_guard_current());
        else
            hipLaunchKernelGGL(sg_attention_bf16x3_p_kernel, dim3(nqb * heads * B2), dim3(512), 0, (hipStream_t)stream, q, k, v, ld, N, heads, B2, n_tok, cross,
                               scale_log2e, out, ldo);
    } else {
        const int nqb = (N + AT_QW * AT_WAVES - 1) / (AT_QW * AT_WAVES);
        hipLaunchKernelGGL(sg_attention_kernel, dim3(nqb * heads * B2), dim3(256), 0, (hipStream_t)stream, q, k, v, ld, N, heads, B2, n_tok, cross,
                           scale_log2e, out, ldo);
    }
    CHECK_LAUNCH();
    return 0;
}

int mfr_sg_attention(const float *q, const float *k, const float *v, int ld, int B2, int N, int heads,
                     const int32_t *n_tok, int cross, float *out, int ldo, void *stream)
{
    return mfr_sg_attention_variant(q, k, v, ld, B2, N, heads, n_tok, cross, out, ldo, 0, stream);
}

}
```

map-free-reloc_amd/csrc/superglue_match.hip:

```cpp
#include <hip/hip_runtime.h>
#include <math.h>
#include <stdint.h>

#include "../../include/mfr_hip.h"
#include "wave_dev.h"
#include "zero_fill.h"

using namespace mfr;

#define SG_LDV(ldS) (((ldS) + 4) & ~3)

struct Lse { float m, s; };
static __device__ __forceinline__ void lse_add(Lse &a, float x)
{
    const float nm = fmaxf(a.m, x);
    a.s = __builtin_fmaf(a.s, __expf(a.m - nm), __expf(x - nm));
    a.m = nm;
}
static __device__ __forceinline__ void lse_merge(Lse &a, float m, float s)
{
    const float nm = fmaxf(a.m, m);
    const float t = s * __expf(m - nm);
    const float ns = __builtin_fmaf(a.s, __expf(a.m - nm), t);
    const bool keep = m == -INFINITY;
    a.s = keep ? a.s : ns;
    a.m = keep ? a.m : nm;
}
static __device__ __forceinline__ float lse_val(const Lse &a) { return a.m + __logf(a.s); }
static __device__ __forceinline__ void lse_block4(float x0, float x1, float x2, float x3, float &bm, float &bs)
{
    bm = fmaxf(fmaxf(x0, x1), fmaxf(x2, x3));
    bs = ((__expf(x0 - bm) + __expf(x1 - bm)) + __expf(x2 - bm)) + __expf(x3 - bm);
}
static __device__ __forceinline__ void lse_merge_block(Lse &a, float bm, float bs)
{
    const float nm = fmaxf(a.m, bm);
    a.s = __builtin_fmaf(a.s, __expf(a.m - nm), bs * __expf(bm - nm));
    a.m = nm;
}
static __device__ __forceinline__ void lse_add4(Lse &a, float x0, float x1, float x2, float x3)
{
    float bm, bs;
    lse_block4(x0, x1, x2, x3, bm, bs);
    lse_merge_block(a, bm, bs);
}
static __device__ __forceinline__ float sg_row_u(const float (&x)[16], float vn, float log_mu, int lane)
{
    float mx = x[0];
#pragma unroll
    for (int k = 1; k < 16; ++k) mx = fmaxf(mx, x[k]);
    mx = fmaxf(wave_max_dpp(mx), vn);
    float sum = 0.f;
#pragma unroll
    for (int k = 0; k < 16; ++k) sum += __expf(x[k] - mx);
    const float sd = sum + __expf(vn - mx);
    sum = wave_sum_dpp(lane == 0 ? sd : sum);
    return log_mu - (mx + __logf(sum));
}
static __device__ __forceinline__ int sg_nq(int m, int g) { return (m - 48 - g > 0) ? (m - 48 - g + 63) / 64 : 0; }
static __device__ __forceinline__ int sg_ntail(int m, int g, int nq) { return max(0, (m - (g + 64 * nq) + 15) / 16); }
static __device__ __forceinline__ int sg_row_of(int g, int r, int nq, int t) { return t < nq ? g + 64 * t + 16 * r : g + 64 * nq + 16 * (t - nq); }

__global__ void __launch_bounds__(256) sg_row_kernel(const float *__restrict__ S, int ldS, const int *__restrict__ n0,
                                                     const int *__restrict__ n1, float alpha,
                                                     const float *__restrict__ v ,
                                                     float *__restrict__ u )
{
    const int b = blockIdx.y, lane = threadIdx.x & 63;
    const int i = blockIdx.x * 4 + (threadIdx.x >> 6);
    const int m = n0[b], n = n1[b];
    if (i > m || m == 0 || n == 0) return;
    const float *vb = v + (size_t)b * SG_LDV(ldS);
    const float norm = -__logf((float)(m + n));
    Lse a = { -INFINITY, 0.f };
    if (i < m && !(ldS & 3) && ldS <= 1024) {
        const float4 *row4 = (const float4 *)(S + ((size_t)b * ldS + i) * ldS), *v4 = (const float4 *)vb;
        float x[16];
#pragma unroll
        for (int k = 0; k < 4; ++k) {
            const int j4 = lane + 64 * k;
            float4 r = make_float4(-INFINITY, -INFINITY, -INFINITY, -INFINITY), w = make_float4(0.f, 0.f, 0.f, 0.f);
            if (4 * j4 < n) { r = row4[j4]; w = v4[j4]; }
            x[4 * k] = (4 * j4 < n) ? r.x + w.x : -INFINITY;
            x[4 * k + 1] = (4 * j4 + 1 < n) ? r.y + w.y : -INFINITY;
            x[4 * k + 2] = (4 * j4 + 2 < n) ? r.z + w.z : -INFINITY;
            x[4 * k + 3] = (4 * j4 + 3 < n) ? r.w + w.w : -INFINITY;
        }
        const float ui = sg_row_u(x, alpha + vb[n], norm, lane);
        if (lane == 0) u[(size_t)b * SG_LDV(ldS) + i] = ui;
        return;
    } else if (i < m) {
        const float *row = S + ((size_t)b * ldS + i) * ldS;
        for (int j = lane; j < n; j += 64) lse_add(a, row[j] + vb[j]);
    } else {
        for (int j = lane; j < n; j += 64) lse_add(a, alpha + vb[j]);
    }
    if (lane == 0) lse_add(a, alpha + vb[n]);
#pragma unroll
    for (int off = 32; off >= 1; off >>= 1) {
        const float om = __shfl_xor(a.m, off, 64), os = __shfl_xor(a.s, off, 64);
        lse_merge(a, om, os);
    }
    if (lane == 0) {
        const float log_mu = (i < m) ? norm : (__logf((float)n) + norm);
        u[(size_t)b * SG_LDV(ldS) + i] = log_mu - lse_val(a);
    }
}

__global__ void __launch_bounds__(1024) sg_col_kernel(const float *__restrict__ S, int ldS, const int *__restrict__ n0,
                                                      const int *__restrict__ n1, float alpha,
                                                      const float *__restrict__ u, float *__restrict__ v)
{
    __shared__ float sm[16][64], ss[16][64];
    const int b = blockIdx.y, lane = threadIdx.x & 63, g = threadIdx.x >> 6;
    const int j = blockIdx.x * 64 + lane;
    const int m = n0[b], n = n1[b];
    if (m == 0 || n == 0) return;
    const float *ub = u + (size_t)b * SG_LDV(ldS);
    Lse a = { -INFINITY, 0.f };
    if (j <= n) {
        const bool dust = j == n;
        const float *col = S + (size_t)b * ldS * ldS + (dust ? 0 : j);
        Lse a1 = { -INFINITY, 0.f }, a2 = a1, a3 = a1;
        const int nq = sg_nq(m, g), ntail = sg_ntail(m, g, nq);
        auto run = [&](Lse &ar, int r) {
            const int nr = nq + (r == 0 ? ntail : 0);
            for (int t = 0; t < nr; t += 4) {
                float x[4];
#pragma unroll
                for (int q = 0; q < 4; ++q) {
                    const int i = sg_row_of(g, r, nq, min(t + q, nr - 1));
                    const float xv = (dust ? alpha : col[(size_t)i * ldS]) + ub[i];
                    x[q] = (t + q < nr) ? xv : -INFINITY;
                }
                lse_add4(ar, x[0], x[1], x[2], x[3]);
            }
        };
        run(a, 0); run(a1, 1); run(a2, 2); run(a3, 3);
        lse_merge(a, a1.m, a1.s); lse_merge(a2, a3.m, a3.s); lse_merge(a, a2.m, a2.s);
        if (g == 0) lse_add(a, alpha + ub[m]);
    }
    sm[g][lane] = a.m; ss[g][lane] = a.s;
    __syncthreads();
    if (g == 0 && j <= n) {
        for (int k = 1; k < 16; ++k) lse_merge(a, sm[k][lane], ss[k][lane]);
        const float norm = -__logf((float)(m + n));
        const float log_nu = (j < n) ? norm : (__logf((float)m) + norm);
        v[(size_t)b * SG_LDV(ldS) + j] = log_nu - lse_val(a);
    }
}

__global__ void __launch_bounds__(512, 2) sg_sweep_kernel(const float *__restrict__ S, int ldS, const int *__restrict__ n0, const int *__restrict__ n1,
                                                       float alpha, const float *__restrict__ v, float *__restrict__ u,
                                                       float *__restrict__ part_m , float *__restrict__ part_s)
{
    __shared__ float xm[1][17][64], xs[1][17][64];
    __shared__ float4 am4[4][4][64], as4[4][4][64];
    __shared__ float amd[4][64], asd[4][64];
    __shared__ float um_s;
    __shared__ float4 wsh[256];
    const int b = blockIdx.y, g = blockIdx.x, lane = threadIdx.x & 63, w8 = threadIdx.x >> 6, r = w8 & 3, hb = w8 >> 2;
    const int m = n0[b], n = n1[b];
    if (m == 0 || n == 0) return;
    const int ldv = SG_LDV(ldS);
    const float *vb = v + (size_t)b * ldv;
    float *ub = u + (size_t)b * ldv;
    const float norm = -__logf((float)(m + n));
    const float4 *v4 = (const float4 *)vb;
    const float vn = alpha + vb[n];

    if (g == 0) {
        if (w8 == 0) {
            Lse a = { -INFINITY, 0.f };
            for (int j = lane; j < n; j += 64) lse_add(a, alpha + vb[j]);
            if (lane == 0) lse_add(a, vn);
#pragma unroll
            for (int off = 32; off >= 1; off >>= 1) {
                const float om = __shfl_xor(a.m, off, 64), os = __shfl_xor(a.s, off, 64);
                lse_merge(a, om, os);
            }
            if (lane == 0) { const float um = (__logf((float)n) + norm) - lse_val(a); ub[m] = um; um_s = um; }
        }
        __syncthreads();
    }

    if (hb == 0) {
#pragma unroll
        for (int k = 0; k < 4; ++k) { am4[r][k][lane] = make_float4(-INFINITY, -INFINITY, -INFINITY, -INFINITY); as4[r][k][lane] = make_float4(0.f, 0.f, 0.f, 0.f); }
        amd[r][lane] = -INFINITY; asd[r][lane] = 0.f;
    }
    const int nq = sg_nq(m, g);
    const int nrows = nq + (r == 0 ? sg_ntail(m, g, nq) : 0);
    const int j4max = (ldS >> 2) - 1;
    bool ok[16];
#pragma unroll
    for (int k = 0; k < 16; ++k) ok[k] = 4 * (lane + 64 * (k >> 2)) + (k & 3) < n;
    if (threadIdx.x < 256) wsh[threadIdx.x] = v4[min((int)threadIdx.x, j4max)];
    const int nblk0 = (nq + sg_ntail(m, g, nq) + 3) >> 2;
    __syncthreads();
    for (int it = 0; 2 * it < nblk0; ++it) {
        const int t = 4 * (2 * it + hb);
        const bool have = t < nrows;
        float bm[17], bs[17];
        if (have) {
            float4 cur[4][4];
#pragma unroll
            for (int q = 0; q < 4; ++q) {
                if (t + q < nrows) {
                    const float4 *row4 = (const float4 *)(S + ((size_t)b * ldS + sg_row_of(g, r, nq, t + q)) * ldS);
#pragma unroll
                    for (int k = 0; k < 4; ++k) cur[q][k] = row4[min(lane + 64 * k, j4max)];
                } else {
#pragma unroll
                    for (int k = 0; k < 4; ++k) cur[q][k] = make_float4(0.f, 0.f, 0.f, 0.f);
                }
            }
            float ui[4];
#pragma unroll
            for (int q = 0; q < 4; ++q) {
                ui[q] = -INFINITY;
                if (t + q < nrows) {
                    float x[16];
#pragma unroll
                    for (int k = 0; k < 4; ++k) {
                        const float4 wk = wsh[lane + 64 * k];
                        x[4 * k] = ok[4 * k] ? cur[q][k].x + wk.x : -INFINITY;
                        x[4 * k + 1] = ok[4 * k + 1] ? cur[q][k].y + wk.y : -INFINITY;
                        x[4 * k + 2] = ok[4 * k + 2] ? cur[q][k].z + wk.z : -INFINITY;
                        x[4 * k + 3] = ok[4 * k + 3] ? cur[q][k].w + wk.w : -INFINITY;
                    }
                    ui[q] = sg_row_u(x, vn, norm, lane);
                    if (lane == 0) ub[sg_row_of(g, r, nq, t + q)] = ui[q];
                }
                __builtin_amdgcn_sched_barrier(0);
            }
#pragma unroll
            for (int k = 0; k < 4; ++k) {
                lse_block4(cur[0][k].x + ui[0], cur[1][k].x + ui[1], cur[2][k].x + ui[2], cur[3][k].x + ui[3], bm[4 * k], bs[4 * k]);
                lse_block4(cur[0][k].y + ui[0], cur[1][k].y + ui[1], cur[2][k].y + ui[2], cur[3][k].y + ui[3], bm[4 * k + 1], bs[4 * k + 1]);
                lse_block4(cur[0][k].z + ui[0], cur[1][k].z + ui[1], cur[2][k].z + ui[2], cur[3][k].z + ui[3], bm[4 * k + 2], bs[4 * k + 2]);
                lse_block4(cur[0][k].w + ui[0], cur[1][k].w + ui[1], cur[2][k].w + ui[2], cur[3][k].w + ui[3], bm[4 * k + 3], bs[4 * k + 3]);
                __builtin_amdgcn_sched_barrier(0);
            }
            lse_block4(alpha + ui[0], alpha + ui[1], alpha + ui[2], alpha + ui[3], bm[16], bs[16]);
        }
#pragma unroll
        for (int ph = 0; ph < 2; ++ph) {
            if (have && hb == ph) {
#pragma unroll
                for (int k = 0; k < 4; ++k) {
                    const float4 pm = am4[r][k][lane], ps = as4[r][k][lane];
                    Lse a0 = { pm.x, ps.x }, a1 = { pm.y, ps.y }, a2 = { pm.z, ps.z }, a3 = { pm.w, ps.w };
                    lse_merge_block(a0, bm[4 * k], bs[4 * k]); lse_merge_block(a1, bm[4 * k + 1], bs[4 * k + 1]);
                    lse_merge_block(a2, bm[4 * k + 2], bs[4 * k + 2]); lse_merge_block(a3, bm[4 * k + 3], bs[4 * k + 3]);
                    am4[r][k][lane] = make_float4(a0.m, a1.m, a2.m, a3.m); as4[r][k][lane] = make_float4(a0.s, a1.s, a2.s, a3.s);
                }
                Lse ad = { amd[r][lane], asd[r][lane] };
                lse_merge_block(ad, bm[16], bs[16]);
                amd[r][lane] = ad.m; asd[r][lane] = ad.s;
            }
            __syncthreads();
        }
    }
    __syncthreads();
    Lse acc[17];
    auto fetch = [&](Lse (&d)[17], int rr) {
#pragma unroll
        for (int k = 0; k < 4; ++k) {
            const float4 pm = am4[rr][k][lane], ps = as4[rr][k][lane];
            d[4 * k] = { pm.x, ps.x }; d[4 * k + 1] = { pm.y, ps.y }; d[4 * k + 2] = { pm.z, ps.z }; d[4 * k + 3] = { pm.w, ps.w };
        }
        d[16] = { amd[rr][lane], asd[rr][lane] };
    };
    if (w8 == 2) {
        Lse o[17];
        fetch(acc, 2); fetch(o, 3);
#pragma unroll
        for (int k = 0; k < 17; ++k) lse_merge(acc[k], o[k].m, o[k].s);
#pragma unroll
        for (int k = 0; k < 17; ++k) { xm[0][k][lane] = acc[k].m; xs[0][k][lane] = acc[k].s; }
    } else if (w8 == 0) {
        Lse o[17];
        fetch(acc, 0); fetch(o, 1);
#pragma unroll
        for (int k = 0; k < 17; ++k) lse_merge(acc[k], o[k].m, o[k].s);
    }
    __syncthreads();
    if (w8 == 0) {
#pragma unroll
        for (int k = 0; k < 17; ++k) lse_merge(acc[k], xm[0][k][lane], xs[0][k][lane]);
        if (g == 0) {
            const float xd = alpha + um_s;
#pragma unroll
            for (int k = 0; k < 17; ++k) lse_add(acc[k], xd);
        }
        float *pmr = part_m + ((size_t)b * 16 + g) * ldv, *psr = part_s + ((size_t)b * 16 + g) * ldv;
        float4 *pm = (float4 *)pmr, *ps = (float4 *)psr;
#pragma unroll
        for (int k = 0; k < 4; ++k) {
            const int j4 = lane + 64 * k;
            if (4 * j4 < n) {
                pm[j4] = make_float4(acc[4 * k].m, acc[4 * k + 1].m, acc[4 * k + 2].m, acc[4 * k + 3].m);
                ps[j4] = make_float4(acc[4 * k].s, acc[4 * k + 1].s, acc[4 * k + 2].s, acc[4 * k + 3].s);
            }
        }
        __builtin_amdgcn_s_waitcnt(0);
        if (lane == (n >> 2) % 64) { pmr[n] = acc[16].m; psr[n] = acc[16].s; }
    }
}

__global__ void __launch_bounds__(64) sg_colmerge_kernel(int ldS, const int *__restrict__ n0, const int *__restrict__ n1,
                                                         const float *__restrict__ part_m, const float *__restrict__ part_s, float *__restrict__ v)
{
    const int b = blockIdx.y, j = blockIdx.x * 64 + threadIdx.x;
    const int m = n0[b], n = n1[b];
    if (m == 0 || n == 0 || j > n) return;
    const int ldv = SG_LDV(ldS);
    const float norm = -__logf((float)(m + n));
    const float *pm = part_m + (size_t)b * 16 * ldv + j, *ps = part_s + (size_t)b * 16 * ldv + j;
    float mm[16], sv[16];
#pragma unroll
    for (int k = 0; k < 16; ++k) { mm[k] = pm[(size_t)k * ldv]; sv[k] = ps[(size_t)k * ldv]; }
    Lse a = { mm[0], sv[0] };
#pragma unroll
    for (int k = 1; k < 16; ++k) lse_merge(a, mm[k], sv[k]);
    const float log_nu = (j < n) ? norm : (__logf((float)m) + norm);
    v[(size_t)b * ldv + j] = log_nu - lse_val(a);
}

__global__ void __launch_bounds__(256) sg_rowmax_kernel(const float *__restrict__ S, int ldS,
                                                        const int *__restrict__ n0, const int *__restrict__ n1,
                                                        const float *__restrict__ v, int *__restrict__ idx0,
                                                        float *__restrict__ val0)
{
    const int b = blockIdx.y, lane = threadIdx.x & 63;
    const int i = blockIdx.x * 4 + (threadIdx.x >> 6);
    const int m = n0[b], n = n1[b];
    if (i >= m || n == 0) return;
    const float *row = S + ((size_t)b * ldS + i) * ldS;
    const float *vb = v + (size_t)b * SG_LDV(ldS);
    float best = -INFINITY; int bi = 0x7fffffff;
    for (int j = lane; j < n; j += 64) {
        const float x = row[j] + vb[j];
        if (x > best) { best = x; bi = j; }
    }
    wave_argmax(best, bi);
    if (lane == 0) { idx0[(size_t)b * ldS + i] = bi; val0[(size_t)b * ldS + i] = best; }
}

__global__ void __launch_bounds__(1024) sg_colmax_kernel(const float *__restrict__ S, int ldS,
                                                         const int *__restrict__ n0, const int *__restrict__ n1,
                                                         const float *__restrict__ u, int *__restrict__ idx1)
{
    __shared__ float sb[16][64];
    __shared__ int si[16][64];
    const int b = blockIdx.y, lane = threadIdx.x & 63, g = threadIdx.x >> 6;
    const int j = blockIdx.x * 64 + lane;
    const int m = n0[b], n = n1[b];
    if (m == 0 || n == 0) return;
    const float *ub = u + (size_t)b * SG_LDV(ldS);
    float best = -INFINITY; int bi = 0x7fffffff;
    if (j < n) {
        const float *col = S + (size_t)b * ldS * ldS + j;
        for (int i = g; i < m; i += 16) {
            const float x = col[(size_t)i * ldS] + ub[i];
            if (x > best) { best = x; bi = i; }
        }
    }
    sb[g][lane] = best; si[g][lane] = bi;
    __syncthreads();
    if (g == 0 && j < n) {
        for (int k = 1; k < 16; ++k) {
            const float ob = sb[k][lane]; const int oi = si[k][lane];
            if (ob > best || (ob == best && oi < bi)) { best = ob; bi = oi; }
        }
        idx1[(size_t)b * ldS + j] = bi;
    }
}

__global__ void __launch_bounds__(256) sg_match_kernel(
    int ldS, const int *__restrict__ n0, const int *__restrict__ n1, const float *__restrict__ u,
    const int *__restrict__ idx0, const float *__restrict__ val0, const int *__restrict__ idx1, float thr,
    const float *__restrict__ kpts0, const float *__restrict__ kpts1, int K ,
    int *__restrict__ matches0, float *__restrict__ mscores0, float *__restrict__ pts0, float *__restrict__ pts1,
    int maxN, int *__restrict__ n_corr)
{
    __shared__ Compact256 cs;
    const int b = blockIdx.x, tid = threadIdx.x;
    const int m = n0[b], n = n1[b];
    int total = 0;
    const float norm = (m > 0 && n > 0) ? -__logf((float)(m + n)) : 0.f;
    for (int start = 0; start < ldS; start += 256) {
        const int i = start + tid;
        bool valid = false;
        int j = -1;
        float sc = 0.f;
        if (i < m && n > 0) {
            j = idx0[(size_t)b * ldS + i];
            const bool mutual = idx1[(size_t)b * ldS + j] == i;
            const float z = val0[(size_t)b * ldS + i] + u[(size_t)b * SG_LDV(ldS) + i] - norm;
            sc = mutual ? __expf(z) : 0.f;
            valid = mutual && (sc > thr);
        }
        if (i < ldS) {
            matches0[(size_t)b * ldS + i] = valid ? j : -1;
            mscores0[(size_t)b * ldS + i] = (i < m) ? sc : 0.f;
        }
        const int o = compact256_slot(cs, valid, total);
        if (valid) {
            if (o < maxN) {
                pts0[((size_t)b * maxN + o) * 2] = kpts0[((size_t)b * K + i) * 2];
                pts0[((size_t)b * maxN + o) * 2 + 1] = kpts0[((size_t)b * K + i) * 2 + 1];
                pts1[((size_t)b * maxN + o) * 2] = kpts1[((size_t)b * K + j) * 2];
                pts1[((size_t)b * maxN + o) * 2 + 1] = kpts1[((size_t)b * K + j) * 2 + 1];
            }
        }
    }
    if (tid == 0) n_corr[b] = min(total, maxN);
}

struct SgWs { size_t u, v, idx0, val0, idx1, part_m, part_s, total; };
static SgWs sg_ws_layout(int B, int ldS)
{
    SgWs w; size_t o = 0;
    w.u = o;    o = align_up(o + sizeof(float) * (size_t)B * SG_LDV(ldS), 256);
    w.v = o;    o = align_up(o + sizeof(float) * (size_t)B * SG_LDV(ldS), 256);
    w.idx0 = o; o = align_up(o + sizeof(int) * (size_t)B * ldS, 256);
    w.val0 = o; o = align_up(o + sizeof(float) * (size_t)B * ldS, 256);
    w.idx1 = o; o = align_up(o + sizeof(int) * (size_t)B * ldS, 256);
    w.part_m = o; o = align_up(o + sizeof(float) * (size_t)B * 16 * SG_LDV(ldS), 256);
    w.part_s = o; o = align_up(o + sizeof(float) * (size_t)B * 16 * SG_LDV(ldS), 256);
    w.total = o;
    return w;
}

extern "C" {

size_t mfr_sg_match_workspace_bytes(int B, int ldS)
{
    if (B <= 0 || ldS <= 0) return 0;
    return sg_ws_layout(B, ldS).total;
}

int mfr_sg_sinkhorn_match_variant(const float *S, int B, int ldS, const int32_t *n0, const int32_t *n1,
                                  float bin_score, int iters, float match_thr,
                                  const float *kpts0, const float *kpts1, int K,
                                  void *workspace, size_t workspace_bytes,
                                  int32_t *matches0, float *mscores0, float *pts0, float *pts1, int maxN, int32_t *n_corr,
                                  int variant, void *stream)
{
    if (!S || !n0 || !n1 || !kpts0 || !kpts1 || !workspace || !matches0 || !mscores0 || !pts0 || !pts1 || !n_corr ||
        B <= 0 || ldS <= 0 || K < ldS || maxN <= 0 || iters < 0 || variant < 0 || variant > 1) return MFR_E_ARG;
    const SgWs w = sg_ws_layout(B, ldS);
    if (workspace_bytes < w.total) return MFR_E_WORKSPACE;
    hipStream_t s = (hipStream_t)stream;
    char *ws = (char *)workspace;
    float *u = (float *)(ws + w.u), *v = (float *)(ws + w.v), *val0 = (float *)(ws + w.val0);
    float *part_m = (float *)(ws + w.part_m), *part_s = (float *)(ws + w.part_s);
    int *idx0 = (int *)(ws + w.idx0), *idx1 = (int *)(ws + w.idx1);
    if (mfr_zero_async(ws + w.u, w.idx0 - w.u, s) != hipSuccess) return MFR_E_LAUNCH;
    const bool sweep = variant == 0 && !(ldS & 3) && ldS <= 1024 && !((uintptr_t)S & 15);
    const dim3 rgrid((ldS + 1 + 3) / 4, B), cgrid((ldS + 1 + 63) / 64, B);
    for (int it = 0; it < iters; ++it) {
        if (sweep) {
            hipLaunchKernelGGL(sg_sweep_kernel, dim3(16, B), dim3(512), 0, s, S, ldS, n0, n1, bin_score, v, u, part_m, part_s);
            hipLaunchKernelGGL(sg_colmerge_kernel, cgrid, dim3(64), 0, s, ldS, n0, n1, part_m, part_s, v);
        } else {
            hipLaunchKernelGGL(sg_row_kernel, rgrid, dim3(256), 0, s, S, ldS, n0, n1, bin_score, v, u);
            hipLaunchKernelGGL(sg_col_kernel, cgrid, dim3(1024), 0, s, S, ldS, n0, n1, bin_score, u, v);
        }
    }
    CHECK_LAUNCH();
    hipLaunchKernelGGL(sg_rowmax_kernel, dim3((ldS + 3) / 4, B), dim3(256), 0, s, S, ldS, n0, n1, v, idx0, val0);
    hipLaunchKernelGGL(sg_colmax_kernel, dim3((ldS + 63) / 64, B), dim3(1024), 0, s, S, ldS, n0, n1, u, idx1);
    hipLaunchKernelGGL(sg_match_kernel, dim3(B), dim3(256), 0, s, ldS, n0, n1, u, idx0, val0, idx1, match_thr, kpts0,
                       kpts1, K, matches0, mscores0, pts0, pts1, maxN, n_corr);
    CHECK_LAUNCH();
    return 0;
}

int mfr_sg_sinkhorn_match(const float *S, int B, int ldS, const int32_t *n0, const int32_t *n1,
                          float bin_score, int iters, float match_thr,
                          const float *kpts0, const float *kpts1, int K,
                          void *workspace, size_t workspace_bytes,
                          int32_t *matches0, float *mscores0, float *pts0, float *pts1, int maxN, int32_t *n_corr,
                          void *stream)
{
    return mfr_sg_sinkhorn_match_variant(S, B, ldS, n0, n1, bin_score, iters, match_thr, kpts0, kpts1, K, workspace, workspace_bytes, matches0, mscores0,
                                         pts0, pts1, maxN, n_corr, 0, stream);
}

}
```

map-free-reloc_amd/nets/superglue.py:

```python
import torch
import torch.nn.functional as F

from .. import _lib
from .linear import SplitBatchedNT, SplitLinear


def _fold_bn(w, b, sd, bn):
    g, beta = sd[bn + ".weight"], sd[bn + ".bias"]
    mean, var = sd[bn + ".running_mean"], sd[bn + ".running_var"]
    s = g / torch.sqrt(var + 1e-5)
    return w * s[:, None], (b - mean) * s + beta


def fold_weights(state_dict, n_layers=18):
    sd = {k: v.double() for k, v in state_dict.items()}
    lin = lambda n: sd[n + ".weight"].squeeze(-1)
    f32 = lambda t: t.float().contiguous()
    kenc = []
    for i in range(4):
        w, b = _fold_bn(lin(f"kenc.encoder.{3 * i}"), sd[f"kenc.encoder.{3 * i}.bias"], sd, f"kenc.encoder.{3 * i + 1}")
        kenc.append((f32(w), f32(b)))
    kenc.append((f32(lin("kenc.encoder.12")), f32(sd["kenc.encoder.12.bias"])))
    perm = torch.tensor([(c % 64) * 4 + c // 64 for c in range(256)])
    layers = []
    c = torch.zeros(256, dtype=torch.float64)
    for l in range(n_layers):
        p = f"gnn.layers.{l}"
        wqkv = torch.cat([lin(f"{p}.attn.proj.{j}")[perm] for j in range(3)], 0)
        bqkv = torch.cat([sd[f"{p}.attn.proj.{j}.bias"][perm] for j in range(3)], 0)
        wm, bm = lin(f"{p}.attn.merge")[:, perm], sd[f"{p}.attn.merge.bias"]
        w1, b1 = _fold_bn(lin(f"{p}.mlp.0"), sd[f"{p}.mlp.0.bias"], sd, f"{p}.mlp.1")
        w1x, w1m = w1[:, :256], w1[:, 256:]
        layers.append(dict(wqkv=f32(wqkv), bqkv=f32(bqkv + wqkv @ c), w1=f32(torch.cat([w1x, w1m @ wm], 1)),
                           b1=f32(b1 + w1m @ bm + w1x @ c), w2=f32(lin(f"{p}.mlp.3")), cross=(l % 2 == 1)))
        c = c + sd[f"{p}.mlp.3.bias"]
    wf = lin("final_proj")
    return dict(kenc=kenc, layers=layers, wf=f32(wf), bf=f32(sd["final_proj.bias"] + wf @ c), bin_score=float(sd["bin_score"]))


def superpoint_from_cfg(cfg, device, node):
    from . import weights as WT
    from .superpoint import SuperPointHIP
    sg = cfg.SUPERGLUE
    sd = WT.from_cfg("SuperPoint", cfg, sg.SUPERPOINT_WEIGHTS, lambda: WT.superpoint_state_dict(sg.SYNTHETIC_SEED))
    return SuperPointHIP(sd, device, node.NMS_RADIUS, node.KEYPOINT_THRESHOLD, node.MAX_KEYPOINTS)


def from_cfg(cfg, device):
    from . import weights as WT
    sg = cfg.SUPERGLUE
    sp = superpoint_from_cfg(cfg, device, sg)
    return sp, SuperGlueHIP(WT.from_cfg("SuperGlue", cfg, sg.SUPERGLUE_WEIGHTS, WT.superglue_state_dict), device, sg.SINKHORN_ITERATIONS, sg.MATCH_THRESHOLD)


class SuperGlueHIP:
    def __init__(self, state_dict, device="cuda", sinkhorn_iterations=20, match_threshold=0.2, n_layers=18):
        _lib.load(require_gpu=True)
        self.device = torch.device(device)
        self.iters, self.match_thr = int(sinkhorn_iterations), float(match_threshold)
        from .. import options
        self.att_variant = 0 if options.get("SPLIT") == "f16x2" else 2
        fw = fold_weights(state_dict, n_layers)
        dev = lambda t: t.to(self.device).contiguous()
        self.kenc = [(dev(w), dev(b)) for w, b in fw["kenc"]]
        self.kenc_lin = [SplitLinear(w, b) for w, b in self.kenc[1:]]
        self.layers = [dict(wqkv=dev(L["wqkv"]), bqkv=dev(L["bqkv"]), w1t=dev(L["w1"]).t(), b1=dev(L["b1"]), w2t=dev(L["w2"]).t(),
                            cross=L["cross"]) for L in fw["layers"]]
        for L in self.layers:
            L["lin_qkv"] = SplitLinear(L["wqkv"], L["bqkv"])
            L["lin1"] = SplitLinear(L["w1t"].t(), L["b1"])
            L["lin2"] = SplitLinear(L["w2t"].t())
        self.wf, self.bf = dev(fw["wf"]), dev(fw["bf"])
        self.lin_final = SplitLinear(self.wf, self.bf)
        self.score_gemm = SplitBatchedNT() if self.lin_final.split == "f16x2" else None
        self.bin_score = fw["bin_score"]
        self._ws = None
        self._size = {}

    def attention(self, qkv, n_tok, cross, out=None, ldo=256, variant=None):
        lib = _lib.load()
        if variant is None:
            variant = self.att_variant
        B2, K, _ = qkv.shape
        if out is None:
            out = torch.empty(B2, K, 256, dtype=torch.float32, device=qkv.device)
        base = qkv.data_ptr()
        _lib.check(lib.mfr_sg_attention_variant(base, base + 256 * 4, base + 512 * 4, 768, B2, K, 4, _lib.ptr(n_tok),
                                                1 if cross else 0, out.data_ptr(), ldo, int(variant), _lib.stream_ptr()), "mfr_sg_attention")
        return out

    def sinkhorn_match(self, S, n0, n1, kpts0, kpts1, maxN=None, variant=0):
        lib = _lib.load()
        B, ldS, _ = S.shape
        K = kpts0.shape[1]
        maxN = maxN or ldS
        dev = S.device
        need = lib.mfr_sg_match_workspace_bytes(B, ldS)
        if self._ws is None or self._ws.numel() < need:
            self._ws = torch.empty(need, dtype=torch.uint8, device=dev)
        m0 = torch.empty(B, ldS, dtype=torch.int32, device=dev)
        ms0 = torch.empty(B, ldS, dtype=torch.float32, device=dev)
        pts0 = torch.zeros(B, maxN, 2, dtype=torch.float32, device=dev)
        pts1 = torch.zeros(B, maxN, 2, dtype=torch.float32, device=dev)
        nc = torch.empty(B, dtype=torch.int32, device=dev)
        _lib.check(lib.mfr_sg_sinkhorn_match_variant(
            _lib.ptr(S.contiguous()), B, ldS, _lib.ptr(n0), _lib.ptr(n1), self.bin_score, self.iters, self.match_thr,
            _lib.ptr(kpts0.contiguous()), _lib.ptr(kpts1.contiguous()), K, _lib.ptr(self._ws), self._ws.numel(),
            _lib.ptr(m0), _lib.ptr(ms0), _lib.ptr(pts0), _lib.ptr(pts1), maxN, _lib.ptr(nc), int(variant), _lib.stream_ptr()),
            "mfr_sg_sinkhorn_match")
        return dict(matches0=m0, matching_scores0=ms0, pts0=pts0, pts1=pts1, n_corr=nc)

    @torch.no_grad()
    def final_descriptors(self, kpts, scores, desc, n, image_hw):
        H, W = image_hw
        B2, K, _ = kpts.shape
        key = (H, W, kpts.device)
        if key not in self._size:
            self._size[key] = torch.tensor([float(W), float(H)], device=kpts.device)
        size = self._size[key]
        kn = (kpts - size / 2) / (float(max(W, H)) * 0.7)
        w0, b0 = self.kenc[0]
        h = (kn[..., 0:1] * w0[:, 0] + kn[..., 1:2] * w0[:, 1]) + (scores.unsqueeze(-1) * w0[:, 2] + b0)
        h = F.relu_(h).reshape(B2 * K, -1)
        for i, lin in enumerate(self.kenc_lin):
            h = lin(h, relu=i < len(self.kenc_lin) - 1)
        xa = torch.empty(B2 * K, 512, dtype=torch.float32, device=kpts.device)
        xv, av = xa[:, :256], xa[:, 256:]
        torch.add(desc.reshape(B2 * K, 256), h.reshape(B2 * K, 256), out=xv)
        qkv = torch.empty(B2 * K, 768, dtype=torch.float32, device=kpts.device)
        hid = torch.empty(B2 * K, 512, dtype=torch.float32, device=kpts.device)
        for L in self.layers:
            L["lin_qkv"](xv, out=qkv)
            self.attention(qkv.view(B2, K, 768), n, L["cross"], out=av, ldo=512)
            L["lin1"](xa, out=hid, relu=True)
            L["lin2"](hid, out=xv, accumulate=True)
        return self.lin_final(xv).view(B2, K, 256)

    @torch.no_grad()
    def __call__(self, sp_out, image_hw, maxN=None):
        kpts, scores, desc, n = sp_out["kpts"], sp_out["scores"], sp_out["desc"], sp_out["n"]
        md = self.final_descriptors(kpts, scores, desc, n, image_hw)
        if self.score_gemm is not None:
            S = self.score_gemm(md[0::2], md[1::2], out_mul=1.0 / 16.0)
        else:
            S = torch.bmm(md[0::2], md[1::2].transpose(1, 2)) * (1.0 / 16.0)
        return self.sinkhorn_match(S, n[0::2].contiguous(), n[1::2].contiguous(),
                                   kpts[0::2].contiguous(), kpts[1::2].contiguous(), maxN)
```

map-free-reloc_amd/options.py:

```python
_SPEC = {
    "SPLIT": ("f16x2", ("f16x2", "bf16x3")),
    "CONV": ("wino", ("wino", "miopen")),
    "CONV_KERNEL": ("auto", ("auto", "split", "exact", "direct")),
    "CONV_TILE": ("auto", ("auto", "rows", "linear")),
    "FUSED_CONV1": (True, (False, True)),
    "FUSED_CONV_RELU": (False, (False, True)),
    "RPR_CONV": ("hip", ("hip", "miopen")),
    "RPR_CONV_BWD": ("lib", ("lib", "hip")),
    "RPR_CONV_ORDER": ("tap_inner", ("tap_inner", "tap_outer")),
    "RPR_WGRAD_SPLITS": (16, None),
    "RPR_ENCODER_NHWC": (False, (False, True)),
}
_VALUES = {k: v[0] for k, v in _SPEC.items()}
_EXPLICIT = set()


def names():
    return sorted(_SPEC)


def default(name):
    return _SPEC[name][0]


def get(name):
    return _VALUES[name]


def set(name, value):
    if name not in _SPEC:
        raise KeyError(f"unknown HIP option {name!r}; known: {names()}")
    dflt, allowed = _SPEC[name]
    if isinstance(dflt, bool):
        if isinstance(value, str):
            value = value.lower() in ("1", "true", "yes", "on")
        value = bool(value)
    elif isinstance(dflt, int):
        value = int(value)
        if value < 1:
            raise ValueError(f"HIP option {name}: must be >= 1")
    if allowed is not None and value not in allowed:
        raise ValueError(f"HIP option {name}={value!r}: allowed {allowed}")
    _VALUES[name] = value
    _EXPLICIT.add(name)


class override:

    def __init__(self, **kv):
        self.kv = kv

    def __enter__(self):
        self.saved = {k: (_VALUES[k], k in _EXPLICIT) for k in self.kv}
        for k, v in self.kv.items():
            set(k, v)
        return self

    def __exit__(self, *exc):
        for k, (v, ex) in self.saved.items():
            _VALUES[k] = v
            (_EXPLICIT.add if ex else _EXPLICIT.discard)(k)
        return False


def reset():
    for k, v in _SPEC.items():
        _VALUES[k] = v[0]
    _EXPLICIT.clear()


def apply_cfg(cfg):
    hip = cfg.HIP if "HIP" in cfg else {}
    for k in _SPEC:
        if k in hip:
            if k in _EXPLICIT and hip[k] == _SPEC[k][0]:
                continue
            explicit = k in _EXPLICIT
            set(k, hip[k])
            if not explicit:
                _EXPLICIT.discard(k)
```

Measured before the change: 1329.

## Process multiple query blocks per attention workgroup and add fused Sinkhorn kernel option

The attention kernel now lets one workgroup loop over several query blocks for the same batch-head. K/V tiles are prefetched cyclically across iterations, the next Q block is loaded during the last tile, and the previous output is stored lazily. By default the number of query blocks per workgroup is chosen to spread work over 256 CUs, which cuts redundant K/V loads and launch waves, at the cost of fewer workgroups and more register pressure. A fused Sinkhorn variant merges the column step into the sweep kernel using last-arriver tickets, but it is opt-in and not the default.

```diff
diff --git a/include/mfr_hip.h b/include/mfr_hip.h
--- a/include/mfr_hip.h
+++ b/include/mfr_hip.h
@@ -160,6 +160,10 @@
                      const int32_t *n_tok, int cross, float *out, int ldo, void *stream);
 int mfr_sg_attention_variant(const float *q, const float *k, const float *v, int ld, int B2, int N, int heads,
                              const int32_t *n_tok, int cross, float *out, int ldo, int variant, void *stream);
+#define MFR_ATT_QBLOCKS_AUTO 0
+#define MFR_ATT_QBLOCKS_XCD (-1)
+int mfr_sg_attention_qblocks(const float *q, const float *k, const float *v, int ld, int B2, int N, int heads,
+                             const int32_t *n_tok, int cross, float *out, int ldo, int variant, int qblocks, void *stream);
 size_t mfr_sg_match_workspace_bytes(int B, int ldS);
 int mfr_sg_sinkhorn_match(const float *S, int B, int ldS, const int32_t *n0, const int32_t *n1,
                           float bin_score, int iters, float match_thr,
diff --git a/map-free-reloc_amd/_lib.py b/map-free-reloc_amd/_lib.py
--- a/map-free-reloc_amd/_lib.py
+++ b/map-free-reloc_amd/_lib.py
@@ -59,6 +59,7 @@
     "mfr_gemm_bf16x3": (_i, [_vp, _i, _vp, _vp, _vp, _i, _i, _i, _i, _i, _vp]),
     "mfr_sg_attention": (_i, [_vp, _vp, _vp, _i, _i, _i, _i, _vp, _i, _vp, _i, _vp]),
     "mfr_sg_attention_variant": (_i, [_vp, _vp, _vp, _i, _i, _i, _i, _vp, _i, _vp, _i, _i, _vp]),
+    "mfr_sg_attention_qblocks": (_i, [_vp, _vp, _vp, _i, _i, _i, _i, _vp, _i, _vp, _i, _i, _i, _vp]),
     "mfr_sg_match_workspace_bytes": (_sz, [_i, _i]),
     "mfr_sg_sinkhorn_match": (_i, [_vp, _i, _i, _vp, _vp, C.c_float, _i, C.c_float, _vp, _vp, _i, _vp, _sz,
                                    _vp, _vp, _vp, _vp, _i, _vp, _vp]),
diff --git a/map-free-reloc_amd/csrc/attention.hip b/map-free-reloc_amd/csrc/attention.hip
--- a/map-free-reloc_amd/csrc/attention.hip
+++ b/map-free-reloc_amd/csrc/attention.hip
@@ -143,8 +143,10 @@
 #define AB_KS 72
 #define AB_VS 40
 #define AB_WAVES 8
+#define AT_CUS 256
 
 typedef float at_f2 __attribute__((ext_vector_type(2)));
+typedef float at_f4 __attribute__((ext_vector_type(4)));
 union Frag8 { bf16x8 v; unsigned u[4]; uint4 q; };
 
 #define MFMA_BF16(a, b, c) __builtin_amdgcn_mfma_f32_32x32x16_bf16((a).v, (b).v, (c), 0, 0, 0)
@@ -186,43 +188,56 @@
 
 template <class AR>
 __device__ __forceinline__ void sg_attention_split_p(
-    const float *Q, const float *Kp, const float *Vp, int ld, int N, int heads, int B2, const int *n_tok, int cross, float scale_log2e, float *O, int ldo, int *guard)
+    const float *Q, const float *Kp, const float *Vp, int ld, int N, int heads, int B2, const int *n_tok, int cross, float scale_log2e, float *O, int ldo, int *guard,
+    int qpw, int xmap)
 {
     constexpr int NT = AR::NT, NO = AR::NO;
     __shared__ __attribute__((aligned(16))) unsigned short Ks[2][NT][AT_KT][AB_KS];
     __shared__ __attribute__((aligned(16))) unsigned short Vt[2][NT][AT_D][AB_VS];
     const int nbh = heads * B2;
-    const int bh = blockIdx.x % nbh, qb = blockIdx.x / nbh;
+    const int nqb = (N + AT_QW * AB_WAVES - 1) / (AT_QW * AB_WAVES), ngroups = (nqb + qpw - 1) / qpw;
+    int bh, qg;
+    if (xmap) { const int j = blockIdx.x >> 3; bh = 8 * (j / ngroups) + (blockIdx.x & 7); qg = j % ngroups; }
+    else { bh = blockIdx.x % nbh; qg = blockIdx.x / nbh; }
+    const int qb0 = qg * qpw, qbe = min(qb0 + qpw, nqb);
     const int b = bh / heads, h = bh - b * heads;
     const int bk = cross ? (b ^ 1) : b;
     const int tid = threadIdx.x, lane = tid & 63, wid = __builtin_amdgcn_readfirstlane(tid >> 6);
     const int ql = lane & 31, half = lane >> 5;
     const int nq = n_tok[b], nk = n_tok[bk];
-    const int q0 = qb * (AT_QW * AB_WAVES);
-    const int q = q0 + wid * AT_QW + ql;
-    if (q0 >= nq) {
-        if (q < N) at_store_zero_row(O + ((size_t)b * N + q) * ldo + h * AT_D + 32 * half);
-        return;
-    }
+    const int qrow = wid * AT_QW + ql;
+    auto zero_blocks = [&](int qb) {
+        for (; qb < qbe; ++qb) {
+            const int q = qb * (AT_QW * AB_WAVES) + qrow;
+            if (q < N) at_store_zero_row(O + ((size_t)b * N + q) * ldo + h * AT_D + 32 * half);
+        }
+    };
+    if (qb0 * (AT_QW * AB_WAVES) >= nq || nk == 0) { zero_blocks(qb0); return; }
 
     Frag8 qf[4][NT];
-    {
+    at_f4 qraw[8];
+    auto gload_q = [&](int q) {
         const bool ok = q < N;
         const float *qp = Q + ((size_t)b * N + (ok ? q : 0)) * ld + h * AT_D + half * 8;
 #pragma unroll
+        for (int s = 0; s < 4; ++s) { qraw[2 * s] = *(const at_f4 *)(qp + 16 * s); qraw[2 * s + 1] = *(const at_f4 *)(qp + 16 * s + 4); }
+    };
+    auto split_q = [&](int q) {
+        const bool ok = q < N;
+        const at_f4 z = { 0.f, 0.f, 0.f, 0.f };
+#pragma unroll
         for (int s = 0; s < 4; ++s) {
-            float4 t0 = *(const float4 *)(qp + 16 * s), t1 = *(const float4 *)(qp + 16 * s + 4);
-            if (!ok) { t0 = make_float4(0.f, 0.f, 0.f, 0.f); t1 = t0; }
+            const at_f4 t0 = ok ? qraw[2 * s] : z, t1 = ok ? qraw[2 * s + 1] : z;
             AR::split2(t0.x * scale_log2e, t0.y * scale_log2e, [&](int k) -> unsigned & { return qf[s][k].u[0]; });
             AR::split2(t0.z * scale_log2e, t0.w * scale_log2e, [&](int k) -> unsigned & { return qf[s][k].u[1]; });
             AR::split2(t1.x * scale_log2e, t1.y * scale_log2e, [&](int k) -> unsigned & { return qf[s][k].u[2]; });
             AR::split2(t1.z * scale_log2e, t1.w * scale_log2e, [&](int k) -> unsigned & { return qf[s][k].u[3]; });
         }
-    }
+    };
+    gload_q(qb0 * (AT_QW * AB_WAVES) + qrow);
+    __builtin_amdgcn_sched_barrier(0);
     f32x16 o0, o1, c0, c1;
-#pragma unroll
-    for (int r = 0; r < 16; ++r) { o0[r] = 0.f; o1[r] = 0.f; c0[r] = 0.f; c1[r] = 0.f; }
-    float m_run = -INFINITY, l_run = 0.f;
+    float m_run, l_run;
 
     const int sr = tid >> 4, sc4 = (tid & 15) * 4;
     const unsigned rowb = (unsigned)ld * 4u;
@@ -231,6 +246,7 @@
     const __amdgpu_buffer_rsrc_t rv = __builtin_amdgcn_make_buffer_rsrc((void *)(Vp + (size_t)bk * N * ld + h * AT_D), 0, (int)span, MFR_RSRC_FLAGS);
     const unsigned koff = (unsigned)sr * rowb + 4u * (unsigned)sc4, voff = 4u * (unsigned)lane;
     const int ntiles = (nk + AT_KT - 1) / AT_KT;
+    auto next_tile = [&](int t) { return t + 1 == ntiles ? 0 : t + 1; };
     float4 kr;
     float v0, v1, v2, v3;
     auto gload_k = [&](int t) { kr = __builtin_bit_cast(float4, __builtin_amdgcn_raw_buffer_load_b128(rk, koff, (unsigned)(t * AT_KT) * rowb, 0)); };
@@ -275,26 +291,39 @@
 #define AT_FOLD_SCORES(sc, s, s2) do { _Pragma("unroll") for (int r_ = 0; r_ < 16; ++r_) sc[r_] = AR::fold(s[r_], s2[r_]); } while (0)
 
     f32x16 sc;
+    const int t1 = next_tile(0), t2 = next_tile(t1);
     gload_k(0); gload_v(0); lstore_k(0); lstore_v(0);
-    gload_k(1); lstore_k(1);
-    gload_k(2); gload_v(1);
+    gload_k(t1); lstore_k(1);
+    gload_k(t2); gload_v(t1);
+    int tk = next_tile(t2), tv = t2, buf = 0;
+    float *op_prev = nullptr;
+    float inv_prev = 0.f;
     __syncthreads();
+
+  for (int qb = qb0;;) {
+    const int q = qb * (AT_QW * AB_WAVES) + qrow;
+    split_q(q);
     {
         f32x16 s, s2;
 #pragma unroll
         for (int r = 0; r < 16; ++r) { s[r] = 0.f; s2[r] = 0.f; }
-        if (ntiles > 0) {
-#pragma unroll
-            for (int st = 0; st < 4; ++st) { Frag8 kf[NT]; AT_KLOAD(kf, kq0, st); AT_QK(kf, qf[st], s, s2); }
-        }
+        const unsigned short *kqp = kq0 + buf * (NT * AT_KT * AB_KS);
+#pragma unroll
+        for (int st = 0; st < 4; ++st) { Frag8 kf[NT]; AT_KLOAD(kf, kqp, st); AT_QK(kf, qf[st], s, s2); }
         AT_FOLD_SCORES(sc, s, s2);
     }
     __syncthreads();
+    if (op_prev) at_store_normalised(op_prev, o0, o1, inv_prev);
+#pragma unroll
+    for (int r = 0; r < 16; ++r) { o0[r] = 0.f; o1[r] = 0.f; c0[r] = 0.f; c1[r] = 0.f; }
+    m_run = -INFINITY; l_run = 0.f;
+    const int qbn = qb + 1;
+    const bool more = qbn < qbe && qbn * (AT_QW * AB_WAVES) < nq;
 
     for (int t = 0; t < ntiles; ++t) {
-        const int buf = t & 1;
         const unsigned short *kq = kq0 + (buf ^ 1) * (NT * AT_KT * AB_KS);
         const unsigned short *vq = vq0 + buf * (NT * AT_D * AB_VS);
+        if (more && t == ntiles - 1) gload_q(qbn * (AT_QW * AB_WAVES) + qrow);
         f32x16 s, s2;
 #pragma unroll
         for (int r = 0; r < 16; ++r) { s[r] = 0.f; s2[r] = 0.f; }
@@ -359,7 +388,8 @@
         Frag8 pf0[NT];
         AT_SPLIT_P(pf0, 0);
         lstore_k(buf); lstore_v(buf ^ 1);
-        gload_k(t + 3); gload_v(t + 2);
+        gload_k(tk); gload_v(tv);
+        tk = next_tile(tk); tv = next_tile(tv);
         AT_WEAVE(6, 14);
         __builtin_amdgcn_sched_barrier(0);
         AT_PV(va, pf0);
@@ -372,7 +402,36 @@
         AT_PV(vb, pf1);
         AT_FOLD_SCORES(sc, s, s2);
         __syncthreads();
-    }
+        buf ^= 1;
+    }
+
+    float *op = nullptr;
+    float inv = 0.f;
+    if (q < N) {
+        inv = (l_run > 0.f && q < nq) ? 1.f / l_run : 0.f;
+        op = O + ((size_t)b * N + q) * ldo + h * AT_D + 4 * half;
+        if constexpr (AR::GUARD) {
+            if (guard) {
+                float chk = 0.f;
+#pragma unroll
+                for (int r = 0; r < 16; ++r) { MFR_GUARD_ACC(chk, o0[r]); MFR_GUARD_ACC(chk, c0[r]); MFR_GUARD_ACC(chk, o1[r]); MFR_GUARD_ACC(chk, c1[r]); }
+                MFR_GUARD_ACC(chk, l_run);
+                if (chk != chk) atomicOr(guard, 1);
+            }
+        }
+        if constexpr (NO == 2) {
+#pragma unroll
+            for (int r = 0; r < 16; ++r) { o0[r] = AR::fold(o0[r], c0[r]); o1[r] = AR::fold(o1[r], c1[r]); }
+        }
+    }
+    if (!more) {
+        if (op) at_store_normalised(op, o0, o1, inv);
+        zero_blocks(qbn);
+        break;
+    }
+    op_prev = op; inv_prev = inv;
+    qb = qbn;
+  }
 #undef AT_FOLD_SCORES
 #undef AT_SPLIT_P
 #undef AT_PV
@@ -380,59 +439,45 @@
 #undef AT_WEAVE
 #undef AT_VLOAD
 #undef AT_KLOAD
-
-    if (q < N) {
-        const float inv = (l_run > 0.f && q < nq) ? 1.f / l_run : 0.f;
-        float *op = O + ((size_t)b * N + q) * ldo + h * AT_D + 4 * half;
-        if constexpr (AR::GUARD) {
-            if (guard) {
-                float chk = 0.f;
-#pragma unroll
-                for (int r = 0; r < 16; ++r) { MFR_GUARD_ACC(chk, o0[r]); MFR_GUARD_ACC(chk, c0[r]); MFR_GUARD_ACC(chk, o1[r]); MFR_GUARD_ACC(chk, c1[r]); }
-                MFR_GUARD_ACC(chk, l_run);
-                if (chk != chk) atomicOr(guard, 1);
-            }
-        }
-        if constexpr (NO == 2) {
-#pragma unroll
-            for (int r = 0; r < 16; ++r) { o0[r] = AR::fold(o0[r], c0[r]); o1[r] = AR::fold(o1[r], c1[r]); }
-        }
-        at_store_normalised(op, o0, o1, inv);
-    }
 }
 
 __global__ void __launch_bounds__(512, 1) sg_attention_bf16x3_p_kernel(
     const float *__restrict__ Q, const float *__restrict__ Kp, const float *__restrict__ Vp, int ld,
-    int N, int heads, int B2, const int *__restrict__ n_tok, int cross, float scale_log2e, float *__restrict__ O, int ldo)
-{
-    sg_attention_split_p<AtBf16x3>(Q, Kp, Vp, ld, N, heads, B2, n_tok, cross, scale_log2e, O, ldo, nullptr);
+    int N, int heads, int B2, const int *__restrict__ n_tok, int cross, float scale_log2e, float *__restrict__ O, int ldo, int qpw, int xmap)
+{
+    sg_attention_split_p<AtBf16x3>(Q, Kp, Vp, ld, N, heads, B2, n_tok, cross, scale_log2e, O, ldo, nullptr, qpw, xmap);
 }
 
 __global__ void __launch_bounds__(512, 1) sg_attention_f16x2_p_kernel(
     const float *__restrict__ Q, const float *__restrict__ Kp, const float *__restrict__ Vp, int ld,
-    int N, int heads, int B2, const int *__restrict__ n_tok, int cross, float scale_log2e, float *__restrict__ O, int ldo, int *guard)
-{
-    sg_attention_split_p<AtF16x2>(Q, Kp, Vp, ld, N, heads, B2, n_tok, cross, scale_log2e, O, ldo, guard);
+    int N, int heads, int B2, const int *__restrict__ n_tok, int cross, float scale_log2e, float *__restrict__ O, int ldo, int *guard, int qpw, int xmap)
+{
+    sg_attention_split_p<AtF16x2>(Q, Kp, Vp, ld, N, heads, B2, n_tok, cross, scale_log2e, O, ldo, guard, qpw, xmap);
 }
 
 extern "C" {
 
-int mfr_sg_attention_variant(const float *q, const float *k, const float *v, int ld, int B2, int N, int heads,
-                             const int32_t *n_tok, int cross, float *out, int ldo, int variant, void *stream)
+int mfr_sg_attention_qblocks(const float *q, const float *k, const float *v, int ld, int B2, int N, int heads,
+                             const int32_t *n_tok, int cross, float *out, int ldo, int variant, int qblocks, void *stream)
 {
     if (!q || !k || !v || !n_tok || !out || B2 <= 0 || N <= 0 || heads <= 0 || (ld & 3) || (ldo & 3)) return MFR_E_ARG;
     if (cross && (B2 & 1)) return MFR_E_ARG;
-    if (variant < 0 || variant > 2) return MFR_E_ARG;
+    if (variant < 0 || variant > 2 || qblocks < MFR_ATT_QBLOCKS_XCD) return MFR_E_ARG;
     if (variant != 1 && (size_t)N * ld * 4 >= 0x7fffffffull) variant = 1;
     const float scale_log2e = 1.4426950408889634f / 8.0f;
     if (variant != 1) {
         const int nqb = (N + AT_QW * AB_WAVES - 1) / (AT_QW * AB_WAVES);
+        const long long nbh = (long long)heads * B2;
+        const int xmap = qblocks == MFR_ATT_QBLOCKS_XCD && nbh % 8 == 0;
+        long long qpw = qblocks == MFR_ATT_QBLOCKS_AUTO ? nqb * nbh / AT_CUS : (qblocks > 0 ? qblocks : 1);
+        qpw = qpw < 1 ? 1 : (qpw > nqb ? nqb : qpw);
+        const unsigned grid = (unsigned)(((nqb + qpw - 1) / qpw) * nbh);
         if (variant == 0)
-            hipLaunchKernelGGL(sg_attention_f16x2_p_kernel, dim3(nqb * heads * B2), dim3(512), 0, (hipStream_t)stream, q, k, v, ld, N, heads, B2, n_tok, cross,
-                               scale_log2e, out, ldo, mfr_guard_current());
+            hipLaunchKernelGGL(sg_attention_f16x2_p_kernel, dim3(grid), dim3(512), 0, (hipStream_t)stream, q, k, v, ld, N, heads, B2, n_tok, cross,
+                               scale_log2e, out, ldo, mfr_guard_current(), (int)qpw, xmap);
         else
-            hipLaunchKernelGGL(sg_attention_bf16x3_p_kernel, dim3(nqb * heads * B2), dim3(512), 0, (hipStream_t)stream, q, k, v, ld, N, heads, B2, n_tok, cross,
-                               scale_log2e, out, ldo);
+            hipLaunchKernelGGL(sg_attention_bf16x3_p_kernel, dim3(grid), dim3(512), 0, (hipStream_t)stream, q, k, v, ld, N, heads, B2, n_tok, cross,
+                               scale_log2e, out, ldo, (int)qpw, xmap);
     } else {
         const int nqb = (N + AT_QW * AT_WAVES - 1) / (AT_QW * AT_WAVES);
         hipLaunchKernelGGL(sg_attention_kernel, dim3(nqb * heads * B2), dim3(256), 0, (hipStream_t)stream, q, k, v, ld, N, heads, B2, n_tok, cross,
@@ -442,6 +487,12 @@
     return 0;
 }
 
+int mfr_sg_attention_variant(const float *q, const float *k, const float *v, int ld, int B2, int N, int heads,
+                             const int32_t *n_tok, int cross, float *out, int ldo, int variant, void *stream)
+{
+    return mfr_sg_attention_qblocks(q, k, v, ld, B2, N, heads, n_tok, cross, out, ldo, variant, MFR_ATT_QBLOCKS_AUTO, stream);
+}
+
 int mfr_sg_attention(const float *q, const float *k, const float *v, int ld, int B2, int N, int heads,
                      const int32_t *n_tok, int cross, float *out, int ldo, void *stream)
 {
diff --git a/map-free-reloc_amd/csrc/superglue_match.hip b/map-free-reloc_amd/csrc/superglue_match.hip
--- a/map-free-reloc_amd/csrc/superglue_match.hip
+++ b/map-free-reloc_amd/csrc/superglue_match.hip
@@ -150,9 +150,37 @@
     }
 }
 
+static __device__ __forceinline__ void sg_fold_v(int j, int m, int n, int ldv, const float *pm , const float *ps, float *vb)
+{
+    const float norm = -__logf((float)(m + n));
+    float mm[16], sv[16];
+#pragma unroll
+    for (int k = 0; k < 16; ++k) { mm[k] = pm[(size_t)k * ldv + j]; sv[k] = ps[(size_t)k * ldv + j]; }
+    Lse a = { mm[0], sv[0] };
+#pragma unroll
+    for (int k = 1; k < 16; ++k) lse_merge(a, mm[k], sv[k]);
+    const float log_nu = (j < n) ? norm : (__logf((float)m) + norm);
+    vb[j] = log_nu - lse_val(a);
+}
+static __device__ __forceinline__ bool sg_last_arriver(int *counter, int target)
+{
+    __shared__ int last_s;
+    asm volatile("s_waitcnt vmcnt(0)" ::: "memory");
+    __syncthreads();
+    if (threadIdx.x == 0) {
+        __builtin_amdgcn_fence(__ATOMIC_RELEASE, "agent");
+        const int last = __hip_atomic_fetch_add(counter, 1, __ATOMIC_RELAXED, __HIP_MEMORY_SCOPE_AGENT) + 1 == target;
+        if (last) __builtin_amdgcn_fence(__ATOMIC_ACQUIRE, "agent");
+        asm volatile("s_waitcnt vmcnt(0)" ::: "memory");
+        last_s = last;
+    }
+    __syncthreads();
+    return last_s != 0;
+}
+
 __global__ void __launch_bounds__(512, 2) sg_sweep_kernel(const float *__restrict__ S, int ldS, const int *__restrict__ n0, const int *__restrict__ n1,
-                                                       float alpha, const float *__restrict__ v, float *__restrict__ u,
-                                                       float *__restrict__ part_m , float *__restrict__ part_s)
+                                                       float alpha, float *v, float *__restrict__ u,
+                                                       float *__restrict__ part_m , float *__restrict__ part_s, int *ticket, int target)
 {
     __shared__ float xm[1][17][64], xs[1][17][64];
     __shared__ float4 am4[4][4][64], as4[4][4][64];
@@ -307,6 +335,10 @@
         __builtin_amdgcn_s_waitcnt(0);
         if (lane == (n >> 2) % 64) { pmr[n] = acc[16].m; psr[n] = acc[16].s; }
     }
+    if (ticket == nullptr) return;
+    if (!sg_last_arriver(ticket + b, target)) return;
+    const float *pm = part_m + (size_t)b * 16 * ldv, *ps = part_s + (size_t)b * 16 * ldv;
+    for (int j = threadIdx.x; j <= n; j += 512) sg_fold_v(j, m, n, ldv, pm, ps, v + (size_t)b * ldv);
 }
 
 __global__ void __launch_bounds__(64) sg_colmerge_kernel(int ldS, const int *__restrict__ n0, const int *__restrict__ n1,
@@ -316,16 +348,7 @@
     const int m = n0[b], n = n1[b];
     if (m == 0 || n == 0 || j > n) return;
     const int ldv = SG_LDV(ldS);
-    const float norm = -__logf((float)(m + n));
-    const float *pm = part_m + (size_t)b * 16 * ldv + j, *ps = part_s + (size_t)b * 16 * ldv + j;
-    float mm[16], sv[16];
-#pragma unroll
-    for (int k = 0; k < 16; ++k) { mm[k] = pm[(size_t)k * ldv]; sv[k] = ps[(size_t)k * ldv]; }
-    Lse a = { mm[0], sv[0] };
-#pragma unroll
-    for (int k = 1; k < 16; ++k) lse_merge(a, mm[k], sv[k]);
-    const float log_nu = (j < n) ? norm : (__logf((float)m) + norm);
-    v[(size_t)b * ldv + j] = log_nu - lse_val(a);
+    sg_fold_v(j, m, n, ldv, part_m + (size_t)b * 16 * ldv, part_s + (size_t)b * 16 * ldv, v + (size_t)b * ldv);
 }
 
 __global__ void __launch_bounds__(256) sg_rowmax_kernel(const float *__restrict__ S, int ldS,
@@ -372,6 +395,78 @@
     if (g == 0 && j < n) {
         for (int k = 1; k < 16; ++k) {
             const float ob = sb[k][lane]; const int oi = si[k][lane];
+            if (ob > best || (ob == best && oi < bi)) { best = ob; bi = oi; }
+        }
+        idx1[(size_t)b * ldS + j] = bi;
+    }
+}
+
+__global__ void __launch_bounds__(512) sg_argmax_kernel(const float *__restrict__ S, int ldS, const int *__restrict__ n0, const int *__restrict__ n1,
+                                                        const float *__restrict__ v, const float *__restrict__ u, int *__restrict__ idx0,
+                                                        float *__restrict__ val0, int *idx1, float *part_b , int *part_i, int *ticket)
+{
+    __shared__ float sb[8][16][64];
+    __shared__ int si[8][16][64];
+    const int b = blockIdx.y, g = blockIdx.x, lane = threadIdx.x & 63, w8 = threadIdx.x >> 6;
+    const int m = n0[b], n = n1[b];
+    if (m == 0 || n == 0) return;
+    const int ldv = SG_LDV(ldS), j4max = (ldS >> 2) - 1;
+    const float *ub = u + (size_t)b * ldv;
+    const float4 *v4 = (const float4 *)(v + (size_t)b * ldv);
+    float4 vv[4];
+#pragma unroll
+    for (int k = 0; k < 4; ++k) vv[k] = v4[min(lane + 64 * k, j4max)];
+    float cb[16]; int ci[16];
+#pragma unroll
+    for (int k = 0; k < 16; ++k) { cb[k] = -INFINITY; ci[k] = 0x7fffffff; }
+    const int nrows = (m - g + 15) / 16;
+    auto one_row = [&](int i, const float4 (&row)[4]) {
+        const float ui = ub[i];
+        float best = -INFINITY; int bi = 0x7fffffff;
+#pragma unroll
+        for (int k = 0; k < 4; ++k) {
+            const float s4[4] = { row[k].x, row[k].y, row[k].z, row[k].w }, w4[4] = { vv[k].x, vv[k].y, vv[k].z, vv[k].w };
+#pragma unroll
+            for (int c = 0; c < 4; ++c) {
+                const int j = 4 * (lane + 64 * k) + c;
+                const float x = s4[c] + w4[c];
+                if (j < n && x > best) { best = x; bi = j; }
+                const float y = s4[c] + ui;
+                if (y > cb[4 * k + c]) { cb[4 * k + c] = y; ci[4 * k + c] = i; }
+            }
+        }
+        wave_argmax(best, bi);
+        if (lane == 0) { idx0[(size_t)b * ldS + i] = bi; val0[(size_t)b * ldS + i] = best; }
+    };
+    for (int t = w8; t < nrows; t += 16) {
+        const int ia = g + 16 * t, ib = ia + 16 * 8;
+        const bool hb = t + 8 < nrows;
+        const float4 *ra = (const float4 *)(S + ((size_t)b * ldS + ia) * ldS), *rb = (const float4 *)(S + ((size_t)b * ldS + (hb ? ib : ia)) * ldS);
+        float4 a4[4], b4[4];
+#pragma unroll
+        for (int k = 0; k < 4; ++k) { a4[k] = ra[min(lane + 64 * k, j4max)]; b4[k] = rb[min(lane + 64 * k, j4max)]; }
+        one_row(ia, a4);
+        if (hb) one_row(ib, b4);
+    }
+#pragma unroll
+    for (int k = 0; k < 16; ++k) { sb[w8][k][lane] = cb[k]; si[w8][k][lane] = ci[k]; }
+    __syncthreads();
+    for (int s = threadIdx.x; s < 1024; s += 512) {
+        const int k = s >> 6, l = s & 63, j = 4 * (l + 64 * (k >> 2)) + (k & 3);
+        float best = sb[0][k][l]; int bi = si[0][k][l];
+#pragma unroll
+        for (int w = 1; w < 8; ++w) {
+            const float ob = sb[w][k][l]; const int oi = si[w][k][l];
+            if (ob > best || (ob == best && oi < bi)) { best = ob; bi = oi; }
+        }
+        if (j < n) { part_b[((size_t)b * 16 + g) * ldv + j] = best; part_i[((size_t)b * 16 + g) * ldv + j] = bi; }
+    }
+    if (!sg_last_arriver(ticket + b, 16)) return;
+    for (int j = threadIdx.x; j < n; j += 512) {
+        const float *pb = part_b + (size_t)b * 16 * ldv + j; const int *pi = part_i + (size_t)b * 16 * ldv + j;
+        float best = pb[0]; int bi = pi[0];
+        for (int k = 1; k < 16; ++k) {
+            const float ob = pb[(size_t)k * ldv]; const int oi = pi[(size_t)k * ldv];
             if (ob > best || (ob == best && oi < bi)) { best = ob; bi = oi; }
         }
         idx1[(size_t)b * ldS + j] = bi;
@@ -419,12 +514,13 @@
     if (tid == 0) n_corr[b] = min(total, maxN);
 }
 
-struct SgWs { size_t u, v, idx0, val0, idx1, part_m, part_s, total; };
+struct SgWs { size_t u, v, ticket, idx0, val0, idx1, part_m, part_s, total; };
 static SgWs sg_ws_layout(int B, int ldS)
 {
     SgWs w; size_t o = 0;
     w.u = o;    o = align_up(o + sizeof(float) * (size_t)B * SG_LDV(ldS), 256);
     w.v = o;    o = align_up(o + sizeof(float) * (size_t)B * SG_LDV(ldS), 256);
+    w.ticket = o; o = align_up(o + sizeof(int) * (size_t)B * 2, 256);
     w.idx0 = o; o = align_up(o + sizeof(int) * (size_t)B * ldS, 256);
     w.val0 = o; o = align_up(o + sizeof(float) * (size_t)B * ldS, 256);
     w.idx1 = o; o = align_up(o + sizeof(int) * (size_t)B * ldS, 256);
@@ -450,7 +546,7 @@
                                   int variant, void *stream)
 {
     if (!S || !n0 || !n1 || !kpts0 || !kpts1 || !workspace || !matches0 || !mscores0 || !pts0 || !pts1 || !n_corr ||
-        B <= 0 || ldS <= 0 || K < ldS || maxN <= 0 || iters < 0 || variant < 0 || variant > 1) return MFR_E_ARG;
+        B <= 0 || ldS <= 0 || K < ldS || maxN <= 0 || iters < 0 || variant < 0 || variant > 2) return MFR_E_ARG;
     const SgWs w = sg_ws_layout(B, ldS);
     if (workspace_bytes < w.total) return MFR_E_WORKSPACE;
     hipStream_t s = (hipStream_t)stream;
@@ -458,12 +554,16 @@
     float *u = (float *)(ws + w.u), *v = (float *)(ws + w.v), *val0 = (float *)(ws + w.val0);
     float *part_m = (float *)(ws + w.part_m), *part_s = (float *)(ws + w.part_s);
     int *idx0 = (int *)(ws + w.idx0), *idx1 = (int *)(ws + w.idx1);
+    int *ticket = (int *)(ws + w.ticket);
     if (mfr_zero_async(ws + w.u, w.idx0 - w.u, s) != hipSuccess) return MFR_E_LAUNCH;
-    const bool sweep = variant == 0 && !(ldS & 3) && ldS <= 1024 && !((uintptr_t)S & 15);
+    const bool sweep = variant != 1 && !(ldS & 3) && ldS <= 1024 && !((uintptr_t)S & 15);
+    const bool fused = sweep && variant == 2;
     const dim3 rgrid((ldS + 1 + 3) / 4, B), cgrid((ldS + 1 + 63) / 64, B);
     for (int it = 0; it < iters; ++it) {
-        if (sweep) {
-            hipLaunchKernelGGL(sg_sweep_kernel, dim3(16, B), dim3(512), 0, s, S, ldS, n0, n1, bin_score, v, u, part_m, part_s);
+        if (fused) {
+            hipLaunchKernelGGL(sg_sweep_kernel, dim3(16, B), dim3(512), 0, s, S, ldS, n0, n1, bin_score, v, u, part_m, part_s, ticket, 16 * (it + 1));
+        } else if (sweep) {
+            hipLaunchKernelGGL(sg_sweep_kernel, dim3(16, B), dim3(512), 0, s, S, ldS, n0, n1, bin_score, v, u, part_m, part_s, (int *)nullptr, 0);
             hipLaunchKernelGGL(sg_colmerge_kernel, cgrid, dim3(64), 0, s, ldS, n0, n1, part_m, part_s, v);
         } else {
             hipLaunchKernelGGL(sg_row_kernel, rgrid, dim3(256), 0, s, S, ldS, n0, n1, bin_score, v, u);
@@ -471,8 +571,12 @@
         }
     }
     CHECK_LAUNCH();
-    hipLaunchKernelGGL(sg_rowmax_kernel, dim3((ldS + 3) / 4, B), dim3(256), 0, s, S, ldS, n0, n1, v, idx0, val0);
-    hipLaunchKernelGGL(sg_colmax_kernel, dim3((ldS + 63) / 64, B), dim3(1024), 0, s, S, ldS, n0, n1, u, idx1);
+    if (fused) {
+        hipLaunchKernelGGL(sg_argmax_kernel, dim3(16, B), dim3(512), 0, s, S, ldS, n0, n1, v, u, idx0, val0, idx1, part_m, (int *)part_s, ticket + B);
+    } else {
+        hipLaunchKernelGGL(sg_rowmax_kernel, dim3((ldS + 3) / 4, B), dim3(256), 0, s, S, ldS, n0, n1, v, idx0, val0);
+        hipLaunchKernelGGL(sg_colmax_kernel, dim3((ldS + 63) / 64, B), dim3(1024), 0, s, S, ldS, n0, n1, u, idx1);
+    }
     hipLaunchKernelGGL(sg_match_kernel, dim3(B), dim3(256), 0, s, ldS, n0, n1, u, idx0, val0, idx1, match_thr, kpts0,
                        kpts1, K, matches0, mscores0, pts0, pts1, maxN, n_corr);
     CHECK_LAUNCH();
diff --git a/map-free-reloc_amd/nets/superglue.py b/map-free-reloc_amd/nets/superglue.py
--- a/map-free-reloc_amd/nets/superglue.py
+++ b/map-free-reloc_amd/nets/superglue.py
@@ -3,6 +3,9 @@
 
 from .. import _lib
 from .linear import SplitBatchedNT, SplitLinear
+
+ATT_QBLOCKS = {"auto": 0, "1": 1, "2": 2, "4": 4, "xcd": -1}
+SINKHORN_KERNEL = {"auto": 0, "sweep": 0, "twopass": 1, "fused": 2}
 
 
 def _fold_bn(w, b, sd, bn):
@@ -85,12 +88,17 @@
         if out is None:
             out = torch.empty(B2, K, 256, dtype=torch.float32, device=qkv.device)
         base = qkv.data_ptr()
-        _lib.check(lib.mfr_sg_attention_variant(base, base + 256 * 4, base + 512 * 4, 768, B2, K, 4, _lib.ptr(n_tok),
-                                                1 if cross else 0, out.data_ptr(), ldo, int(variant), _lib.stream_ptr()), "mfr_sg_attention")
+        from .. import options
+        qblocks = ATT_QBLOCKS[options.get("ATT_QBLOCKS")]
+        _lib.check(lib.mfr_sg_attention_qblocks(base, base + 256 * 4, base + 512 * 4, 768, B2, K, 4, _lib.ptr(n_tok),
+                                                1 if cross else 0, out.data_ptr(), ldo, int(variant), qblocks, _lib.stream_ptr()), "mfr_sg_attention")
         return out
 
-    def sinkhorn_match(self, S, n0, n1, kpts0, kpts1, maxN=None, variant=0):
+    def sinkhorn_match(self, S, n0, n1, kpts0, kpts1, maxN=None, variant=None):
         lib = _lib.load()
+        if variant is None:
+            from .. import options
+            variant = SINKHORN_KERNEL[options.get("SINKHORN_KERNEL")]
         B, ldS, _ = S.shape
         K = kpts0.shape[1]
         maxN = maxN or ldS
diff --git a/map-free-reloc_amd/options.py b/map-free-reloc_amd/options.py
--- a/map-free-reloc_amd/options.py
+++ b/map-free-reloc_amd/options.py
@@ -3,6 +3,8 @@
     "CONV": ("wino", ("wino", "miopen")),
     "CONV_KERNEL": ("auto", ("auto", "split", "exact", "direct")),
     "CONV_TILE": ("auto", ("auto", "rows", "linear")),
+    "ATT_QBLOCKS": ("auto", ("auto", "1", "2", "4", "xcd")),
+    "SINKHORN_KERNEL": ("auto", ("auto", "sweep", "twopass", "fused")),
     "FUSED_CONV1": (True, (False, True)),
     "FUSED_CONV_RELU": (False, (False, True)),
     "RPR_CONV": ("hip", ("hip", "miopen")),
@@ -39,6 +41,8 @@
         value = int(value)
         if value < 1:
             raise ValueError(f"HIP option {name}: must be >= 1")
+    elif isinstance(value, int) and not isinstance(value, bool):
+        value = str(value)
     if allowed is not None and value not in allowed:
         raise ValueError(f"HIP option {name}={value!r}: allowed {allowed}")
     _VALUES[name] = value
```

New measurement: 1330, median of 3. About the same (+0.0%).
